# brianz98/A-Fortran-Electronic-Structure-Program

Measured on AMD Instinct MI355X. Metric: CCSD iter wall-time (s) + (T) wall-time (s); fp64 TFLOP/s vs MFMA peak, higher is better.
Workload: dtype f64; 1 GPU; cfg5: nocc=20 nvirt=200, synthetic hashed ERIs scale 0.005; step = 1 CCSD iteration (replicated) + full (T) over i<=j<=k sharded across ranks; nocc=20, nvirt=200, triples=1540, parallelism=(T) ijk-shard x1, CCSD replicas

## Files before the change

### a-fortran-electronic-structure-program_amd/afesp_amd/capi.py

```python
from __future__ import annotations

import ctypes as C
import os

import numpy as np

_HERE = os.path.dirname(os.path.abspath(__file__))
LIB_PATH = os.environ.get("AFESP_LIBRARY") or os.path.join(os.path.dirname(_HERE), "csrc", "libafesp_hip.so")

i64 = C.c_int64
dbl = C.c_double
_dp = np.ctypeslib.ndpointer(dtype=np.float64, flags="C_CONTIGUOUS")
_opt = C.c_void_p

EXPORTS = [
    "afesp_ctx_create", "afesp_ctx_destroy", "afesp_last_error", "afesp_version", "afesp_neri", "afesp_ao2mo_mp2",
    "afesp_ccsd_init", "afesp_ccsd_iterate", "afesp_ccsd_energy", "afesp_ccsd_diis", "afesp_ccsd_solve",
    "afesp_ccsd_get_amplitudes", "afesp_ccsd_set_amplitudes", "afesp_ccsd_get_tensor", "afesp_ccsd_update_intermediates",
    "afesp_ccsd_update_amplitudes", "afesp_ccsd_t_ntriples", "afesp_ccsd_t", "afesp_ccsd_t_shard_bounds", "afesp_gemm", "afesp_permute4",
    "afesp_contract", "afesp_synthetic_init", "afesp_time_pp_ladder", "afesp_bench_contract", "afesp_set_tuning", "afesp_bench_stream", "afesp_profile", "afesp_ccsd_cr_intermediates", "afesp_ccsd_t_cr",
    "afesp_ccsd_so_init", "afesp_ccsd_so_energy", "afesp_ccsd_so_iterate", "afesp_ccsd_so_diis", "afesp_ccsd_so_get_amplitudes",
    "afesp_ccsd_so_set_amplitudes", "afesp_ccsd_so_get_tensor", "afesp_ccsd_so_t_ntriples", "afesp_ccsd_so_t",
    "afesp_read_eri_text", "afesp_write_fcidump", "afesp_set_eri", "afesp_build_fock", "afesp_ccsd_t_plain",
    "afesp_synthetic_ao", "afesp_ccsd_pp_ladder_flop", "afesp_ccsd_iteration_flop",
    "afesp_device_count", "afesp_comm_unique_id", "afesp_comm_init", "afesp_comm_destroy", "afesp_allreduce_sum",
    "afesp_build_fock_uhf", "afesp_ao2mo_ump2", "afesp_ccsd_uso_init", "afesp_mo_window", "afesp_umo_window",
    "afesp_mp2_vv_density", "afesp_ump2_vv_density",
    "afesp_ccsd_t_block_size", "afesp_test_inject", "afesp_ccsd_is_split", "afesp_ccsd_set_split", "afesp_ccsd_set_fused", "afesp_ccsd_iteration_launches", "afesp_debug_stamps", "afesp_launch_counts", "afesp_first_use_count", "afesp_test_ring_path", "afesp_arena_stats",
]
COMM_RCCL, COMM_HOST = 0, 1


class AfespError(RuntimeError):
    pass


_lib = None


def load_library():
    global _lib
    if _lib is not None:
        return _lib
    if not os.path.exists(LIB_PATH):
        raise AfespError(f"{LIB_PATH} is missing: build it with `make -C {os.path.dirname(LIB_PATH)}` "
                         "(there is no CPU fallback for the accelerated path)")
    L = C.CDLL(LIB_PATH)
    L.afesp_ctx_create.argtypes = [C.c_int, C.POINTER(C.c_void_p)]
    L.afesp_ctx_destroy.argtypes = [C.c_void_p]
    L.afesp_ctx_destroy.restype = None
    L.afesp_last_error.argtypes = [C.c_void_p]
    L.afesp_last_error.restype = C.c_char_p
    L.afesp_neri.argtypes = [i64]
    L.afesp_neri.restype = i64
    L.afesp_ao2mo_mp2.argtypes = [C.c_void_p, i64, i64, _dp, _dp, _opt, _opt, C.POINTER(dbl)]
    L.afesp_ccsd_init.argtypes = [C.c_void_p, i64, i64, _opt, _dp, C.c_int]
    L.afesp_ccsd_iterate.argtypes = [C.c_void_p, dbl, dbl, C.POINTER(dbl), C.POINTER(dbl), C.POINTER(C.c_int)]
    L.afesp_ccsd_energy.argtypes = [C.c_void_p, dbl, dbl, C.POINTER(dbl), C.POINTER(dbl), C.POINTER(C.c_int)]
    L.afesp_ccsd_diis.argtypes = [C.c_void_p]
    L.afesp_ccsd_solve.argtypes = [C.c_void_p, C.c_int, dbl, dbl, _dp, _dp, C.POINTER(C.c_int)]
    L.afesp_ccsd_get_amplitudes.argtypes = [C.c_void_p, _dp, _dp]
    L.afesp_ccsd_set_amplitudes.argtypes = [C.c_void_p, _dp, _dp]
    L.afesp_ccsd_get_tensor.argtypes = [C.c_void_p, C.c_char_p, _dp, i64]
    L.afesp_ccsd_update_intermediates.argtypes = [C.c_void_p]
    L.afesp_ccsd_update_amplitudes.argtypes = [C.c_void_p]
    L.afesp_ccsd_t_ntriples.argtypes = [i64]
    L.afesp_ccsd_t_ntriples.restype = i64
    L.afesp_ccsd_t_shard_bounds.argtypes = [C.c_void_p, i64, i64, C.c_int, C.c_int, C.POINTER(i64)]
    L.afesp_ccsd_t.argtypes = [C.c_void_p, i64, i64, _dp]
    L.afesp_ccsd_t_cr.argtypes = [C.c_void_p, i64, i64, _dp]
    L.afesp_ccsd_t_plain.argtypes = [C.c_void_p, i64, i64, _dp]
    L.afesp_ccsd_cr_intermediates.argtypes = [C.c_void_p]
    L.afesp_gemm.argtypes = [C.c_void_p, C.c_char, C.c_char, i64, i64, i64, dbl, _dp, _dp, dbl, _dp]
    L.afesp_permute4.argtypes = [C.c_void_p, C.POINTER(i64), C.c_char_p, _dp, _dp, C.c_int, dbl]
    L.afesp_contract.argtypes = [C.c_void_p, dbl, _dp, C.c_char_p, C.POINTER(i64), _dp, C.c_char_p, C.POINTER(i64), dbl,
                                 _dp, C.c_char_p, C.POINTER(i64), C.c_int, C.c_int, C.c_int]
    L.afesp_synthetic_init.argtypes = [C.c_void_p, i64, i64, dbl, C.c_uint64, C.c_int]
    L.afesp_time_pp_ladder.argtypes = [C.c_void_p, C.c_int, C.POINTER(dbl)]
    L.afesp_synthetic_ao.argtypes = [C.c_void_p, i64, dbl, C.c_uint64]
    L.afesp_ccsd_pp_ladder_flop.argtypes = [C.c_void_p, C.POINTER(dbl)]
    L.afesp_ccsd_iteration_flop.argtypes = [C.c_void_p, C.POINTER(dbl)]
    L.afesp_bench_contract.argtypes = [C.c_void_p, C.c_char_p, C.POINTER(i64), C.c_char_p, C.POINTER(i64), C.c_char_p,
                                       C.POINTER(i64), C.c_int, C.POINTER(dbl)]
    L.afesp_set_tuning.argtypes = [C.c_int, C.c_int, C.c_int, C.c_int]
    L.afesp_bench_stream.argtypes = [C.c_void_p, i64, C.c_int, C.POINTER(dbl)]
    L.afesp_profile.argtypes = [C.c_void_p, C.c_int, _dp]
    L.afesp_ccsd_so_init.argtypes = [C.c_void_p, i64, i64, _opt, _dp, C.c_int, C.c_int]
    L.afesp_ccsd_so_iterate.argtypes = [C.c_void_p, dbl, dbl, C.POINTER(dbl), C.POINTER(dbl), C.POINTER(C.c_int)]
    L.afesp_ccsd_so_energy.argtypes = [C.c_void_p, dbl, dbl, C.POINTER(dbl), C.POINTER(dbl), C.POINTER(C.c_int)]
    L.afesp_ccsd_so_diis.argtypes = [C.c_void_p]
    L.afesp_ccsd_so_get_amplitudes.argtypes = [C.c_void_p, _dp, _dp]
    L.afesp_ccsd_so_set_amplitudes.argtypes = [C.c_void_p, _dp, _dp]
    L.afesp_ccsd_so_get_tensor.argtypes = [C.c_void_p, C.c_char_p, _dp, i64]
    L.afesp_ccsd_so_t_ntriples.argtypes = [i64]
    L.afesp_ccsd_so_t_ntriples.restype = i64
    L.afesp_ccsd_so_t.argtypes = [C.c_void_p, i64, i64, C.POINTER(dbl)]
    L.afesp_read_eri_text.argtypes = [C.c_void_p, C.c_char_p, i64, _opt, C.POINTER(i64)]
    L.afesp_write_fcidump.argtypes = [C.c_void_p, C.c_char_p, i64, C.POINTER(i64)]
    L.afesp_set_eri.argtypes = [C.c_void_p, i64, _dp]
    L.afesp_build_fock.argtypes = [C.c_void_p, i64, _dp, _dp, _dp]
    L.afesp_build_fock_uhf.argtypes = [C.c_void_p, i64, _dp, _dp, _dp, _dp, _dp]
    L.afesp_ao2mo_ump2.argtypes = [C.c_void_p, i64, i64, i64, _dp, _dp, _dp, _dp, _opt, _opt, _opt, _opt, C.POINTER(dbl)]
    L.afesp_ccsd_uso_init.argtypes = [C.c_void_p, i64, i64, i64, _dp, _dp, C.c_int]
    L.afesp_mo_window.argtypes = [C.c_void_p, i64, i64, i64, i64, _dp, _opt, _opt, C.POINTER(dbl)]
    L.afesp_umo_window.argtypes = [C.c_void_p, i64, i64, i64, i64, i64, _dp, _dp, _opt, _opt, _opt, C.POINTER(dbl)]
    L.afesp_mp2_vv_density.argtypes = [C.c_void_p, i64, i64, i64, _dp, _dp, C.POINTER(dbl)]
    L.afesp_ump2_vv_density.argtypes = [C.c_void_p, i64, i64, i64, i64, _dp, _dp, _dp, _dp, C.POINTER(dbl)]
    L.afesp_device_count.argtypes = []
    L.afesp_comm_unique_id.argtypes = [C.c_char_p]
    L.afesp_comm_init.argtypes = [C.c_void_p, C.c_int, C.c_int, C.c_int, C.c_char_p, C.c_char_p]
    L.afesp_comm_destroy.argtypes = [C.c_void_p]
    L.afesp_allreduce_sum.argtypes = [C.c_void_p, _dp, i64]
    L.afesp_ccsd_t_block_size.argtypes = [C.c_void_p, i64, i64, C.c_int, C.POINTER(C.c_int)]
    L.afesp_test_inject.argtypes = [C.c_void_p, C.c_int]
    L.afesp_arena_stats.argtypes = [C.c_void_p, _dp]
    L.afesp_ccsd_is_split.argtypes = [C.c_void_p, C.POINTER(C.c_int)]
    L.afesp_ccsd_set_split.argtypes = [C.c_void_p, C.c_int]
    L.afesp_ccsd_set_fused.argtypes = [C.c_void_p, C.c_int]
    L.afesp_ccsd_iteration_launches.argtypes = [C.c_void_p, C.POINTER(C.c_int)]
    L.afesp_debug_stamps.argtypes = [C.c_void_p, C.c_int]
    L.afesp_launch_counts.argtypes = [C.c_void_p, C.POINTER(C.c_uint64)]
    L.afesp_first_use_count.argtypes = []
    L.afesp_first_use_count.restype = C.c_uint64
    L.afesp_test_ring_path.argtypes = [C.c_int64, C.c_int64]
    _lib = L
    return L


def _f(a):
    return np.ascontiguousarray(np.asarray(a, dtype=np.float64).ravel(order="F"))


TENSOR_SHAPES = {
    "v_oovv": "oovv", "v_ovov": "ovov", "v_vvov": "vvov", "v_oovo": "oovo", "v_oooo": "oooo", "v_vvvv": "vvvv",
    "I_vo": "vo", "I_vv": "vv", "I_oo_p": "oo", "I_oo": "oo", "c_oovv": "oovv", "asym_t2": "oovv", "x_voov": "voov",
    "I_oooo": "oooo", "I_ovov": "ovov", "I_voov": "voov", "I_vovv_p": "vovv", "I_ooov_p": "ooov", "r1": "ov",
    "r2": "oovv", "D1": "ov", "D2": "oovv", "t1": "ov", "t2": "oovv",
}


def device_count():
    return int(load_library().afesp_device_count())


def first_use_count():
    return int(load_library().afesp_first_use_count())


class Engine:

    def __init__(self, device: int = 0):
        self.L = load_library()
        h = C.c_void_p()
        rc = self.L.afesp_ctx_create(device, C.byref(h))
        if rc != 0:
            raise AfespError(f"afesp_ctx_create(device={device}) failed with status {rc} "
                             "(no usable MI355X/HIP device; the accelerated path has no CPU fallback)")
        self.h = h
        self.o = self.v = 0

    def close(self):
        if getattr(self, "h", None):
            self.L.afesp_ctx_destroy(self.h)
            self.h = None

    def __del__(self):
        self.close()

    def __enter__(self):
        return self

    def __exit__(self, *exc):
        self.close()

    def _chk(self, rc):
        if rc != 0:
            raise AfespError(f"status {rc}: {self.L.afesp_last_error(self.h).decode()}")

    def do_mp2_spatial(self, nbasis, nocc, canon_coeff, canon_levels, eri_packed, want_eri_mo=True):
        e2 = dbl(0.0)
        out = np.zeros(self.L.afesp_neri(nbasis)) if want_eri_mo else None
        src = None
        if eri_packed is not None:
            eri_packed = np.ascontiguousarray(eri_packed, dtype=np.float64)
            src = eri_packed.ctypes.data_as(C.c_void_p)
        self._chk(self.L.afesp_ao2mo_mp2(self.h, nbasis, nocc, _f(canon_coeff), _f(canon_levels), src,
                                         out.ctypes.data_as(C.c_void_p) if out is not None else None, C.byref(e2)))
        return e2.value, out

    def ccsd_init(self, nocc, nvirt, canon_levels, eri_mo_packed=None, diis_n_errmat=8):
        self.o, self.v = int(nocc), int(nvirt)
        ptr = None
        if eri_mo_packed is not None:
            eri_mo_packed = np.ascontiguousarray(eri_mo_packed, dtype=np.float64)
            ptr = eri_mo_packed.ctypes.data_as(C.c_void_p)
        self._chk(self.L.afesp_ccsd_init(self.h, nocc, nvirt, ptr, _f(canon_levels), diis_n_errmat))

    def synthetic_init(self, nocc, nvirt, scale=0.02, seed=12345, diis_n_errmat=8):
        self.o, self.v = int(nocc), int(nvirt)
        self._chk(self.L.afesp_synthetic_init(self.h, nocc, nvirt, scale, seed, diis_n_errmat))

    def ccsd_energy(self, e_tol=1e-6, t_tol=1e-7):
        e, r, c = dbl(), dbl(), C.c_int()
        self._chk(self.L.afesp_ccsd_energy(self.h, e_tol, t_tol, C.byref(e), C.byref(r), C.byref(c)))
# ... 4 lines not shown
        self._chk(self.L.afesp_ccsd_iterate(self.h, e_tol, t_tol, C.byref(e), C.byref(r), C.byref(c)))
        return e.value, r.value, bool(c.value)

    def ccsd_diis(self):
        self._chk(self.L.afesp_ccsd_diis(self.h))

    def update_intermediates(self):
        self._chk(self.L.afesp_ccsd_update_intermediates(self.h))

    def update_amplitudes(self):
        self._chk(self.L.afesp_ccsd_update_amplitudes(self.h))

    def do_ccsd_spatial(self, maxiter=50, e_tol=1e-6, t_tol=1e-7):
        en = np.zeros(maxiter + 1)
        rm = np.zeros(maxiter + 1)
        nit = C.c_int()
        self._chk(self.L.afesp_ccsd_solve(self.h, maxiter, e_tol, t_tol, en, rm, C.byref(nit)))
        return nit.value, en, rm

    def amplitudes(self):
        o, v = self.o, self.v
        t1 = np.zeros(o * v)
        t2 = np.zeros(o * o * v * v)
        self._chk(self.L.afesp_ccsd_get_amplitudes(self.h, t1, t2))
        return t1.reshape((o, v), order="F"), t2.reshape((o, o, v, v), order="F")

    def set_amplitudes(self, t1, t2):
        self._chk(self.L.afesp_ccsd_set_amplitudes(self.h, _f(t1), _f(t2)))

    def tensor(self, name):
        dims = tuple(self.o if ch == "o" else self.v for ch in TENSOR_SHAPES[name])
        buf = np.zeros(int(np.prod(dims)))
        self._chk(self.L.afesp_ccsd_get_tensor(self.h, name.encode(), buf, buf.size))
        return buf.reshape(dims, order="F")

    def ntriples(self):
        return self.L.afesp_ccsd_t_ntriples(self.o)

    def shard_bounds(self, world, cr=False):
        b = (i64 * (world + 1))()
        self._chk(self.L.afesp_ccsd_t_shard_bounds(self.h, self.o, self.v, 1 if cr else 0, world, b))
        return [int(x) for x in b]

    def do_ccsd_t_spatial(self, t_begin=0, t_end=None):
        out = np.zeros(4)
        if t_end is None:
            t_end = self.ntriples()
        self._chk(self.L.afesp_ccsd_t(self.h, t_begin, t_end, out))
        return out

    def comm_unique_id(self) -> bytes:
        buf = C.create_string_buffer(128)
        rc = self.L.afesp_comm_unique_id(buf)
        if rc != 0:
            raise AfespError(f"afesp_comm_unique_id failed with status {rc} (is librccl.so.1 loadable?)")
        return buf.raw

    def comm_init(self, rank, world, transport=COMM_RCCL, bootstrap_path=None, unique_id=None):
        self._chk(self.L.afesp_comm_init(self.h, rank, world, transport,
                                         None if bootstrap_path is None else str(bootstrap_path).encode(), unique_id))

    def comm_destroy(self):
        self._chk(self.L.afesp_comm_destroy(self.h))

    def allreduce_sum(self, values):
        buf = np.ascontiguousarray(values, dtype=np.float64).copy()
        self._chk(self.L.afesp_allreduce_sum(self.h, buf, buf.size))
        return buf

    def t_block_size(self, cr=False):
        sb = C.c_int()
        self._chk(self.L.afesp_ccsd_t_block_size(self.h, self.o, self.v, 1 if cr else 0, C.byref(sb)))
        return sb.value

    def arena_stats(self):
        out = np.zeros(4)
        self._chk(self.L.afesp_arena_stats(self.h, out))
        return dict(driver_calls=int(out[0]), reuse_hits=int(out[1]), idle_gb=out[2] / 1e9, live_gb=out[3] / 1e9)

    def launch_counts(self):
        out = (C.c_uint64 * 4)()
        self._chk(self.L.afesp_launch_counts(self.h, out))
        return dict(tall=int(out[0]), gett=int(out[1]), tgemm=int(out[2]), tgemm_mixed=int(out[3]))

    def ccsd_set_split(self, mode):
        self._chk(self.L.afesp_ccsd_set_split(self.h, int(mode)))

    def ccsd_set_fused(self, mode):
        self._chk(self.L.afesp_ccsd_set_fused(self.h, int(mode)))

    def ccsd_iteration_launches(self):
        n = C.c_int()
        self._chk(self.L.afesp_ccsd_iteration_launches(self.h, C.byref(n)))
        return n.value

    def ccsd_is_split(self):
        f = C.c_int()
        self._chk(self.L.afesp_ccsd_is_split(self.h, C.byref(f)))
        return bool(f.value)

    def test_inject(self, what):
        self._chk(self.L.afesp_test_inject(self.h, what))

    def read_eri_text(self, path, nbasis, want_host_copy=True):
        out = np.zeros(self.L.afesp_neri(nbasis)) if want_host_copy else None
        n = i64()
        self._chk(self.L.afesp_read_eri_text(self.h, str(path).encode(), nbasis,
                                             out.ctypes.data_as(C.c_void_p) if out is not None else None, C.byref(n)))
        return out, n.value

    def set_eri(self, nbasis, eri_packed):
        self._chk(self.L.afesp_set_eri(self.h, nbasis, np.ascontiguousarray(eri_packed, dtype=np.float64)))

    def build_fock(self, nbasis, density, core_hamil):
        out = np.zeros(nbasis * nbasis)
        self._chk(self.L.afesp_build_fock(self.h, nbasis, _f(density), _f(core_hamil), out))
        return out.reshape((nbasis, nbasis), order="F")

    def build_fock_uhf(self, nbasis, dens_a, dens_b, core_hamil):
        fa, fb = np.zeros(nbasis * nbasis), np.zeros(nbasis * nbasis)
        self._chk(self.L.afesp_build_fock_uhf(self.h, nbasis, _f(dens_a), _f(dens_b), _f(core_hamil), fa, fb))
        return fa.reshape((nbasis, nbasis), order="F"), fb.reshape((nbasis, nbasis), order="F")

    def do_ump2(self, nbasis, nalpha, nbeta, coeff_a, coeff_b, levels_a, levels_b, eri_packed=None, want_eri_mo=True):
        e2 = dbl(0.0)
        npr = nbasis * (nbasis + 1) // 2
        aa = np.zeros(self.L.afesp_neri(nbasis)) if want_eri_mo else None
        bb = np.zeros(self.L.afesp_neri(nbasis)) if want_eri_mo else None
        ab = np.zeros(npr * npr) if want_eri_mo else None
        src = None
        if eri_packed is not None:
            eri_packed = np.ascontiguousarray(eri_packed, dtype=np.float64)
            src = eri_packed.ctypes.data_as(C.c_void_p)
        ptr = lambda a: a.ctypes.data_as(C.c_void_p) if a is not None else None
        self._chk(self.L.afesp_ao2mo_ump2(self.h, nbasis, nalpha, nbeta, _f(coeff_a), _f(coeff_b),
                                          np.ascontiguousarray(levels_a, dtype=np.float64), np.ascontiguousarray(levels_b, dtype=np.float64),
                                          src, ptr(aa), ptr(ab), ptr(bb), C.byref(e2)))
        return e2.value, aa, (ab.reshape((npr, npr)) if ab is not None else None), bb

    def init_cc_uspinorb(self, nbasis, nalpha, nbeta, levels_a, levels_b, diis_nerr=8):
        self.so_o = int(nalpha + nbeta)
        self.so_v = int(2 * nbasis - self.so_o)
        self._chk(self.L.afesp_ccsd_uso_init(self.h, nbasis, nalpha, nbeta, np.ascontiguousarray(levels_a, dtype=np.float64),
                                             np.ascontiguousarray(levels_b, dtype=np.float64), diis_nerr))

    def mo_window(self, nbasis, nocc, nfc, nfv, canon_levels, eri_mo=None, want_eri=True):
        e2 = dbl(0.0)
        n_act = int(nbasis) - int(nfc) - int(nfv)
        out = np.zeros(self.L.afesp_neri(n_act)) if want_eri and 0 < n_act <= nbasis else None
        src = None
        if eri_mo is not None:
            eri_mo = np.ascontiguousarray(eri_mo, dtype=np.float64)
            src = eri_mo.ctypes.data_as(C.c_void_p)
        self._chk(self.L.afesp_mo_window(self.h, nbasis, nocc, nfc, nfv, np.ascontiguousarray(canon_levels, dtype=np.float64), src,
                                         out.ctypes.data_as(C.c_void_p) if out is not None else None, C.byref(e2)))
        return out, e2.value

    def umo_window(self, nbasis, nalpha, nbeta, nfc, nfv, levels_a, levels_b, want_eri=True):
        e2 = dbl(0.0)
        n_act = int(nbasis) - int(nfc) - int(nfv)
        ok = want_eri and 0 < n_act <= nbasis
        npr = n_act * (n_act + 1) // 2
        aa = np.zeros(self.L.afesp_neri(n_act)) if ok else None
        bb = np.zeros(self.L.afesp_neri(n_act)) if ok else None
        ab = np.zeros(npr * npr) if ok else None
        ptr = lambda a: a.ctypes.data_as(C.c_void_p) if a is not None else None
# ... 193 lines not shown
```

### a-fortran-electronic-structure-program_amd/csrc/afesp_internal.h

```cpp
#pragma once
#include <hip/hip_runtime.h>
#include <stdint.h>

#include <map>
#include <stdexcept>
#include <string>
#include <thread>
#include <vector>

#include "gett.h"
#include "tgemm.h"

namespace afesp {

struct Error : std::runtime_error {
    int code;
    Error(int c, const std::string& m) : std::runtime_error(m), code(c) {}
};

#define AFESP_HIP(expr)                                                                                    \
    do {                                                                                                   \
        hipError_t e_ = (expr);                                                                            \
        if (e_ != hipSuccess)                                                                              \
            throw ::afesp::Error(2, std::string(#expr) + ": " + hipGetErrorString(e_) + " (" + __FILE__ + \
                                        ":" + std::to_string(__LINE__) + ")");                            \
    } while (0)

struct Tensor {
    double* d = nullptr;
    int rank = 0;
    int64_t dim[6] = {0, 0, 0, 0, 0, 0};
    int64_t stride[6] = {0, 0, 0, 0, 0, 0};
    int64_t frozen = 0;
    int64_t size() const
    {
        int64_t s = 1;
        for (int i = 0; i < rank; ++i) s *= dim[i];
        return s;
    }
};

struct Plan {
    int64_t *offAm, *offAk, *offBk, *offBn, *offCm, *offCn;
    int M, N, K;
    bool swapped, a_kc, b_kc, wide;
    bool a_mu = false, b_nu = false;
    int repack = 0;
    int64_t repack_stride[6] = {0, 0, 0, 0, 0, 0};
    int64_t repack_of = 0, repack_epoch = -1;
    const double* repack_src = nullptr;
};

struct Comm;
struct Recorder;

struct Arena {
    std::map<void*, size_t> live;
    std::multimap<size_t, void*> idle;
    size_t idle_bytes = 0, driver_calls = 0, reuse_hits = 0;
    void* get(size_t bytes);
    void* take_largest(size_t min_bytes, size_t max_bytes, size_t* got);
    void put(void* p);
    void trim();
    void destroy();
};

struct Context {
    int device = 0;
    Comm* comm = nullptr;
    int cc_split_mode = -1;
    int test_throw = 0;
    int fused_mode = -1;
    struct PendingTables { int64_t* dst; std::vector<int64_t> img; };
    std::vector<PendingTables> pending_host;
    std::vector<std::vector<int64_t>> pending_merged;
    void plan_uploads_issue();
    void plan_uploads_done() { pending_host.clear(); pending_merged.clear(); }
    Recorder* rec = nullptr;
    hipStream_t stream = nullptr;
    Arena arena;
    std::vector<void*> owned;
    GettWorkspace ws{nullptr, 0};
    TgLaunchState tg;
    unsigned long long n_tall = 0, n_gett = 0;
    bool in_repack = false;
    GettProblem* capture = nullptr;
    struct Lane {
        hipStream_t stream = nullptr;
        GettWorkspace ws{nullptr, 0};
        hipEvent_t done = nullptr;
    };
    std::vector<Lane> lanes;
    size_t lane_ws_bytes = (size_t)8 << 20;
    struct Prepared {
        std::vector<Lane> lanes;
        void* ws_block = nullptr;
        size_t ws_bytes = 0;
    };
    Prepared prepared;
    std::thread startup;
    static void prepare_lanes(Prepared& out, int nlanes);
    hipEvent_t fork_ev = nullptr;
    int cur_lane = 0;
    void fork(int nlanes);
    void use_lane(int i);
    void join();
    int mark();
    void wait(int mark_id);
    std::vector<hipEvent_t> marks;
    int marks_used = 0;
    double* scal = nullptr;
    double* scal_host = nullptr;
    double* res_host = nullptr;
    double* res_dev = nullptr;
    int64_t res_seq = 0;
    int64_t pub_seq = 0;
    std::map<std::string, Plan> plans;
    size_t plan_bytes = 0;
    std::vector<void*> plan_blocks;
    int64_t* plan_slab = nullptr;
    size_t plan_slab_left = 0;
    int64_t* plan_alloc(size_t n);
    void plan_clear();
    int64_t plan_epoch = 0;
    std::map<std::string, std::pair<void*, size_t>> cache;
    std::string last_error;
    bool prof = false;
    double prof_gemm_ms = 0.0, prof_gemm_flop = 0.0, prof_orbit_ms = 0.0, prof_orbit_bytes = 0.0;
    double prof_gemm_flop_padded = 0.0;
    int prof_gemm_kind = 0;
    int64_t prof_gemm_launches = 0, prof_orbit_launches = 0;

    double* alloc(int64_t n);
    double* alloc_raw(int64_t n);
    int64_t* alloc_i64(int64_t n);
    void release(void* p);
    double* scratch(const std::string& name, int64_t ndoubles);
    void drop_scratch();
    void drop_scratch(const std::string& prefix);
    int64_t scratch_epoch = 0;
    int64_t amp_clock = 0;
    const void* t_ops_owner = nullptr;
    int64_t t_ops_amp = -1, t_ops_scratch = -1, t_ops_cr = -1;
    bool t_ops_ts = false;
    Tensor tensor(std::initializer_list<int64_t> dims);
    void sync();
    void quiesce();
    ~Context();
};

Tensor view(double* d, std::initializer_list<int64_t> dims);

void contract(Context& cx, double alpha, const Tensor& A, const char* la, const Tensor& B, const char* lb, double beta,
              const Tensor& C, const char* lc, int nbatch = 1, const int64_t* bA = nullptr, const int64_t* bB = nullptr,
              const int64_t* bC = nullptr, int force_split = 0, int force_tm = 0, int force_tn = 0);

struct ContractCall {
    double alpha;
    const Tensor* A;
    const char* la;
    const Tensor* B;
    const char* lb;
    double beta;
    const Tensor* C;
    const char* lc;
};
void contract_pair(Context& cx, const ContractCall& c1, const ContractCall& c2);
// ... 95 lines not shown
```

### a-fortran-electronic-structure-program_amd/csrc/capi.hip

```cpp
#include <atomic>
#include <chrono>
#include <mutex>
#include <cstdio>
#include <cstring>
#include <thread>
#include <vector>

#include "../../include/afesp.h"
#include "integrals.h"
#include "ccsd_so.h"
#include "comm.h"
#include "fused.h"
#include "tall.h"

using namespace afesp;

struct afesp_ctx {
    Context cx;
    CCState cc;
    SOState so;
    Integrals in;
    struct GraphSlot {
        hipGraphExec_t exec = nullptr;
        int64_t epoch = -1;
        int calls = 0;
        bool disabled = false;
        void reset()
        {
            if (exec) (void)hipGraphExecDestroy(exec);
            exec = nullptr;
            calls = 0;
            disabled = knobs().no_graph;
        }
    } graph_cc;
    FusedSlot fused_int, fused_amp, fused_iter;
    FusedSlot fused_so;
    void cc_programs_reset()
    {
        graph_cc.reset();
        fused_slot_reset(cx, fused_int);
        fused_slot_reset(cx, fused_amp);
        fused_slot_reset(cx, fused_iter);
    }
    void so_programs_reset() { fused_slot_reset(cx, fused_so); }
};

namespace {

struct PreloadClaim {
    std::mutex mu;
    unsigned long long claimed = 0;
    bool claim(int dev)
    {
        std::lock_guard<std::mutex> lk(mu);
        if (dev < 0 || dev >= 64 || (claimed >> dev) & 1ull) return false;
        claimed |= 1ull << dev;
        return true;
    }
};
PreloadClaim g_preload;

template <class F>
int entry(afesp_ctx* c, F&& f)
{
    if (!c) return 1;
    Context& cx = c->cx;
    first_use_tls_device() = cx.device;
    knobs_refresh();
    auto failed = [&](const char* what, int code) {
        cx.last_error = what;
        if (!cx.lanes.empty()) {
            cx.quiesce();
            cx.use_lane(0);
            cx.marks_used = 0;
        }
        return code ? code : 1;
    };
    try {
        AFESP_HIP(hipSetDevice(cx.device));
        f(cx);
        return 0;
    } catch (const Error& e) {
        return failed(e.what(), e.code);
    } catch (const std::exception& e) {
        return failed(e.what(), 1);
    }
}

template <class Body>
double time_on_stream(Context& cx, int reps, Body body)
{
    struct Event { hipEvent_t e = nullptr; ~Event() { if (e) (void)hipEventDestroy(e); } } a, b;
    AFESP_HIP(hipEventCreate(&a.e));
    AFESP_HIP(hipEventCreate(&b.e));
    body();
    AFESP_HIP(hipEventRecord(a.e, cx.stream));
    for (int r = 0; r < reps; ++r) body();
    AFESP_HIP(hipEventRecord(b.e, cx.stream));
    AFESP_HIP(hipEventSynchronize(b.e));
    float ms = 0.f;
    AFESP_HIP(hipEventElapsedTime(&ms, a.e, b.e));
    return (double)ms / (reps > 0 ? reps : 1);
}

__device__ __forceinline__ double hash_uniform(uint64_t x)
{
    x += 0x9E3779B97F4A7C15ull;
    x = (x ^ (x >> 30)) * 0xBF58476D1CE4E5B9ull;
    x = (x ^ (x >> 27)) * 0x94D049BB133111EBull;
    x ^= x >> 31;
    return (double)(x >> 11) * (1.0 / 9007199254740992.0);
}
__global__ void synth_packed_kernel(double* packed, int64_t n, double scale, uint64_t seed)
{
    for (int64_t k = (int64_t)blockIdx.x * blockDim.x + threadIdx.x; k < n; k += (int64_t)gridDim.x * blockDim.x)
        packed[k] = scale * (2.0 * hash_uniform(seed + (uint64_t)k) - 1.0);
}

}

template <typename Body>
static void replay(afesp_ctx* ctx, afesp_ctx::GraphSlot& g, bool eligible, Body body)
{
    Context& cx = ctx->cx;
    if (g.exec && g.epoch != cx.scratch_epoch) {
        (void)hipGraphExecDestroy(g.exec);
        g.exec = nullptr;
        g.calls = 0;
    }
    if (g.exec) {
        AFESP_HIP(hipGraphLaunch(g.exec, cx.stream));
        return;
    }
    if (!eligible || g.disabled) {
        body();
        return;
    }
    const int graph_after = knobs().graph_after;
    if (g.calls == 0 || g.epoch != cx.scratch_epoch || g.calls < graph_after) {
        body();
        g.calls = (g.epoch != cx.scratch_epoch) ? 1 : g.calls + 1;
        g.epoch = cx.scratch_epoch;
        return;
    }
    cx.use_lane(0);
    hipStream_t origin = cx.stream;
    hipGraph_t graph = nullptr;
    if (hipStreamBeginCapture(origin, hipStreamCaptureModeThreadLocal) != hipSuccess) {
        (void)hipGetLastError();
        g.disabled = true;
// ... 54 lines not shown
    replay(ctx, ctx->graph_cc, ccsd_uses_lanes(ctx->cc), [&] {
        ccsd_intermediates(ctx->cx, ctx->cc, true);
        ccsd_amplitudes(ctx->cx, ctx->cc);
        ccsd_energy_launch(ctx->cx, ctx->cc);
    });
    return false;
}

extern "C" {

int afesp_version(void) { return 1; }
int64_t afesp_neri(int64_t nbasis) { return neri_of(nbasis); }

int afesp_ctx_create(int device, afesp_ctx** out)
{
    if (!out) return 1;
    *out = nullptr;
    int ndev = 0;
    if (hipGetDeviceCount(&ndev) != hipSuccess || ndev <= 0) return 10;
    if (device < 0 || device >= ndev) return 11;
    if (hipSetDevice(device) != hipSuccess) return 12;
    afesp_ctx* c = new afesp_ctx();
    c->cx.device = device;
    int rc = entry(c, [&](Context&) {
        AFESP_HIP(hipStreamCreate(&c->cx.stream));
        c->cx.scal = c->cx.alloc(64 + 18 * 512);
        AFESP_HIP(hipHostMalloc((void**)&c->cx.scal_host, sizeof(double) * 64, hipHostMallocDefault));
        AFESP_HIP(hipHostMalloc((void**)&c->cx.res_host, sizeof(double) * (8 + 256 + 72), hipHostMallocCoherent | hipHostMallocMapped));
        memset(c->cx.res_host, 0, sizeof(double) * (8 + 256 + 72));
        AFESP_HIP(hipHostGetDevicePointer((void**)&c->cx.res_dev, c->cx.res_host, 0));
        c->cx.ws.bytes = (size_t)256 << 20;
        c->cx.ws.ptr = c->cx.alloc((int64_t)(c->cx.ws.bytes / sizeof(double)));
        c->cx.sync();
        if (!knobs().no_preload) {
            if (g_preload.claim(device)) c->cx.startup = std::thread([device, c] {
                first_use_tls_device() = device;
                if (hipSetDevice(device) != hipSuccess) return;
                if (knobs().preload_lanes) Context::prepare_lanes(c->cx.prepared, 6);
                {
                    void* d = nullptr;
                    hipStream_t st = nullptr;
                    std::vector<double> h(4096, 1.0);
                    if (hipStreamCreateWithFlags(&st, hipStreamNonBlocking) == hipSuccess && hipMalloc(&d, h.size() * sizeof(double)) == hipSuccess) {
                        (void)hipMemsetAsync(d, 0, h.size() * sizeof(double), st);
                        (void)hipMemcpyAsync(d, h.data(), h.size() * sizeof(double), hipMemcpyHostToDevice, st);
                        (void)hipMemcpyAsync((char*)d + 8192, d, 8192, hipMemcpyDeviceToDevice, st);
                        (void)hipMemcpyAsync(h.data(), d, h.size() * sizeof(double), hipMemcpyDeviceToHost, st);
                        (void)hipStreamSynchronize(st);
                    }
                    if (d) (void)hipFree(d);
                    if (st) (void)hipStreamDestroy(st);
                    (void)hipGetLastError();
                }
                const bool dbg = knobs().preload_debug;
                auto timed = [dbg](const char* what, void (*fn)()) {
                    const auto t0 = std::chrono::steady_clock::now();
                    fn();
                    if (dbg) fprintf(stderr, "afesp preload %-10s %7.2f ms\n", what, std::chrono::duration<double, std::milli>(std::chrono::steady_clock::now() - t0).count());
                };
                timed("kernels", preload_kernels);
                timed("fused", preload_fused);
                timed("contract", preload_contract);
                timed("small path", preload_small_path_kernels);
                timed("triples", preload_triples);
                timed("ccsd_so", preload_ccsd_so);
                timed("uhf", preload_uhf_kernels);
                if (knobs().preload_gett) timed("gett", preload_gett);
            });
        }
    });
    if (rc) {
        if (c->cx.startup.joinable()) c->cx.startup.join();
        delete c;
        return rc;
    }
    *out = c;
    return 0;
}

void afesp_ctx_destroy(afesp_ctx* ctx)
{
    if (!ctx) return;
    first_use_tls_device() = ctx->cx.device;
    (void)hipSetDevice(ctx->cx.device);
    if (ctx->cx.startup.joinable()) ctx->cx.startup.join();
    ctx->cc_programs_reset();
    ctx->so_programs_reset();
    comm_destroy(ctx->cx.comm);
    ctx->cx.comm = nullptr;
    triples_plan_free(ctx->cc);
    so_triples_plan_free(ctx->so);
    ring_free(ctx->cx, ctx->cc);
    delete ctx;
}

const char* afesp_last_error(const afesp_ctx* ctx) { return ctx ? ctx->cx.last_error.c_str() : "null context"; }

int afesp_ao2mo_mp2(afesp_ctx* ctx, int64_t nbasis, int64_t nocc, const double* canon_coeff, const double* canon_levels,
                    const double* eri_packed, double* eri_mo_packed, double* e_mp2)
{
    return entry(ctx, [&](Context& cx) {
        if (nbasis <= 0 || nocc <= 0 || nbasis - nocc <= 0 || nbasis > 1024) throw Error(1, "afesp_ao2mo_mp2: bad extents");
        const double emp2 = ao2mo_mp2(cx, ctx->in, ctx->cc, nbasis, nocc, canon_coeff, canon_levels, eri_packed, eri_mo_packed);
        if (e_mp2) *e_mp2 = emp2;
    });
}

int afesp_mo_window(afesp_ctx* ctx, int64_t nbasis, int64_t nocc, int64_t n_frozen_core, int64_t n_frozen_virt,
                    const double* canon_levels, const double* eri_mo_packed, double* eri_act, double* e_mp2)
{
    return entry(ctx, [&](Context& cx) {
        const int64_t n = nbasis, nfc = n_frozen_core, nfv = n_frozen_virt;
        if (n <= 0 || n > 1024 || nocc <= 0 || nocc >= n || !canon_levels) throw Error(1, "afesp_mo_window: bad extents");
        if (nfc < 0 || nfv < 0) throw Error(1, "afesp_mo_window: negative number of frozen orbitals");
        if (nfc >= nocc) throw Error(1, "afesp_mo_window: no active occupied orbital left");
        if (nfv >= n - nocc) throw Error(1, "afesp_mo_window: no active virtual orbital left");
        if (!eri_mo_packed && (!ctx->in.mo || ctx->in.mo_n != n))
            throw Error(1, "afesp_mo_window: eri_mo_packed is NULL and no MO integrals are resident for this basis size "
                           "(call afesp_ao2mo_mp2 first; a window is taken once)");
        const double emp2 = mo_window(cx, ctx->in, ctx->cc, n, nocc, nfc, nfv, canon_levels, eri_mo_packed, eri_act);
        if (e_mp2) *e_mp2 = emp2;
    });
}

int afesp_mp2_vv_density(afesp_ctx* ctx, int64_t nbasis, int64_t nocc, int64_t n_frozen_core, const double* canon_levels, double* d_vv,
                         double* e_mp2)
{
    return entry(ctx, [&](Context& cx) {
        const int64_t n = nbasis, nfc = n_frozen_core;
        if (n <= 0 || n > 1024 || nocc <= 0 || nocc >= n || !canon_levels || !d_vv) throw Error(1, "afesp_mp2_vv_density: bad extents");
        if (nfc < 0) throw Error(1, "afesp_mp2_vv_density: negative number of frozen orbitals");
        if (nfc >= nocc) throw Error(1, "afesp_mp2_vv_density: no active occupied orbital left");
        if (!ctx->in.mo || ctx->in.mo_n != n)
            throw Error(1, "afesp_mp2_vv_density: no MO integrals are resident for this basis size (call afesp_ao2mo_mp2 first, and "
                           "afesp_mo_window afterwards)");
        const double emp2 = mp2_vv_density(cx, ctx->in, n, nocc, nfc, canon_levels, d_vv);
        if (e_mp2) *e_mp2 = emp2;
    });
}

int afesp_ccsd_init(afesp_ctx* ctx, int64_t nocc, int64_t nvirt, const double* eri_mo_packed, const double* canon_levels,
                    int diis_n_errmat)
{
    return entry(ctx, [&](Context& cx) {
        const int64_t n = nocc + nvirt;
        if (nocc <= 0 || nvirt <= 0 || n > 1024) throw Error(1, "afesp_ccsd_init: bad extents");
        const double* src = ctx->in.mo;
        double* tmp = nullptr;
        if (eri_mo_packed) {
            if (ccsd_can_reinit(ctx->cc, (int)nocc, (int)nvirt, diis_n_errmat) && ctx->cc.eri_own) {
                cx.quiesce();
                if (ctx->cc.eri_src == ctx->cc.eri_own) ctx->cc.eri_src = nullptr;
                cx.release(ctx->cc.eri_own);
                ctx->cc.eri_own = nullptr;
            }
            tmp = cx.alloc(neri_of(n));
            AFESP_HIP(hipMemcpyAsync(tmp, eri_mo_packed, sizeof(double) * neri_of(n), hipMemcpyHostToDevice, cx.stream));
            src = tmp;
        } else if (!src || ctx->in.mo_n != n) {
            throw Error(1, "afesp_ccsd_init: no MO integrals resident for this basis size (call afesp_ao2mo_mp2 first)");
        }
        if (!ccsd_can_reinit(ctx->cc, (int)nocc, (int)nvirt, diis_n_errmat)) {
            ctx->cc_programs_reset();
            cx.drop_scratch("ao2mo_");
        } else {
            ctx->graph_cc.reset();
// ... 676 lines not shown
        cx.sync();
        comm_destroy(cx.comm);
        cx.comm = nullptr;
        ctx->cc_programs_reset();
    });
}

int afesp_allreduce_sum(afesp_ctx* ctx, double* inout, int64_t n)
{
    return entry(ctx, [&](Context& cx) {
        if (n < 0 || (n > 0 && !inout)) throw Error(1, "afesp_allreduce_sum: bad arguments");
        if (!cx.comm) return;
        comm_allreduce_host(cx, cx.comm, inout, n);
    });
}

int afesp_ccsd_is_split(afesp_ctx* ctx, int* split)
{
    return entry(ctx, [&](Context& cx) {
        if (!ctx->cc.ready || !split) throw Error(1, "afesp_ccsd_is_split: no CCSD state");
        ccsd_refresh_sharding(cx, ctx->cc);
        *split = ctx->cc.sharded ? 1 : 0;
    });
}

int afesp_ccsd_set_fused(afesp_ctx* ctx, int mode)
{
    return entry(ctx, [&](Context& cx) {
        if (mode < -1 || mode > 1) throw Error(1, "afesp_ccsd_set_fused: mode is -1 (environment), 0 (call by call) or 1 (launch-fused)");
        cx.fused_mode = mode;
    });
}

int afesp_ccsd_iteration_launches(afesp_ctx* ctx, int* launches)
{
    return entry(ctx, [&](Context& cx) {
        if (!launches) throw Error(1, "afesp_ccsd_iteration_launches: null argument");
        *launches = fused_launches(ctx->fused_iter.prog);
    });
}

int afesp_ccsd_set_split(afesp_ctx* ctx, int mode)
{
    return entry(ctx, [&](Context& cx) {
        if (mode < -1 || mode > 1) throw Error(1, "afesp_ccsd_set_split: mode is -1 (environment), 0 (replicas) or 1 (split)");
        cx.cc_split_mode = mode;
    });
}

int afesp_ccsd_t_block_size(afesp_ctx* ctx, int64_t nocc, int64_t nvirt, int cr, int* block_size)
{
    return entry(ctx, [&](Context& cx) {
        if (nocc < 1 || nvirt < 1 || !block_size) throw Error(1, "afesp_ccsd_t_block_size: bad arguments");
        *block_size = triples_block_size((int)nocc, (int)nvirt, cr != 0);
    });
}

int afesp_debug_stamps(unsigned long long* out, int n)
{
    knobs_refresh();
    if (n < 0) return triples_read_orbit_stamps(out, -n) == hipSuccess ? 0 : 1;
    if (knobs().stamps_grouped) return gett_read_stamps_grouped(out, n) == hipSuccess ? 0 : 1;
    return gett_read_stamps(out, n) == hipSuccess ? 0 : 1;
}

int afesp_test_ring_path(int64_t nocc, int64_t nvirt)
{
    knobs_refresh();
    CCState s;
    s.o = (int)nocc;
    s.v = (int)nvirt;
    return ring_tg_applies(s) ? 1 : 0;
}

uint64_t afesp_first_use_count(void) { return first_use_count().load(std::memory_order_relaxed); }

int afesp_launch_counts(afesp_ctx* ctx, uint64_t out[4])
{
    return entry(ctx, [&](Context& cx) {
        out[0] = cx.n_tall; out[1] = cx.n_gett; out[2] = cx.tg.launches; out[3] = cx.tg.launches_mixed;
    });
}

int afesp_arena_stats(afesp_ctx* ctx, double out[4])
{
    return entry(ctx, [&](Context& cx) {
        const Arena& a = cx.arena;
        size_t live = 0;
        for (auto& kv : a.live) live += kv.second;
        out[0] = (double)a.driver_calls; out[1] = (double)a.reuse_hits; out[2] = (double)a.idle_bytes; out[3] = (double)live;
    });
}

int afesp_test_inject(afesp_ctx* ctx, int what)
{
    return entry(ctx, [&](Context& cx) { cx.test_throw = what; });
}

}
```

### a-fortran-electronic-structure-program_amd/csrc/ccsd.hip

```cpp
#include <algorithm>
#include <cmath>
#include <cstdlib>
#include <cstring>

#include "ccsd.h"
#include "comm.h"
#include "fused.h"

namespace afesp {

static inline int64_t tri64(int64_t i, int64_t j) { return i >= j ? i * (i + 1) / 2 + j : j * (j + 1) / 2 + i; }

bool ccsd_can_reinit(const CCState& s, int o, int v, int diis_nerr)
{
    if (!knobs().cc_reinit) return false;
    return s.ready && s.o == o && s.v == v && s.nerr == diis_nerr && s.pp_sym == pp_sym_pays(o, v);
}

void ccsd_init(Context& cx, CCState& s, int o, int v, const double* eri_mo_dev, const double* e_host, int diis_nerr)
{
    if (o <= 0 || v <= 0) throw Error(1, "ccsd_init: need at least one occupied and one virtual orbital");
    const bool again = ccsd_can_reinit(s, o, v, diis_nerr);
    if (again) {
        cx.quiesce();
// ... 214 lines not shown
    s.amps_touched = false;
    s.r1x_valid = false;
    int64_t v0, v1;
    slice_bounds(s, &v0, &v1);
    auto sl = [&](const Tensor& t, int axis) { return slice_axis(t, axis, v0, v1); };
    if (!(lanes_pay(s) || cx.rec) && ring_tg_applies(s) && ring_tg_pack(cx, s)) {}
    else k_asym_c(cx, s.asym.d, s.c.d, s.t1.d, s.t2.d, s.o, s.v);
    const bool par = lanes_pay(s) && !cx.rec;
    const bool fused = cx.rec != nullptr;
    const bool ring = !par && !fused && ring_tg_applies(s);
    if (!ring) ring_invalidate(s);
    auto lane = [&](int i) { if (par) cx.use_lane(i); };
    if (par) cx.fork(6);
    lane(0);
    C(1.0, s.w_oovv, "miea", s.t1, "me", 0.0, s.I_vo, "ai");
    lane(1);
    const bool ivv_diag = !par && !fused && s.o >= 2;
    if (!ivv_diag) {
        ccsd_need_w_vvov(cx, s);
        C(1.0, s.w_vvov, "ebma", s.t1, "me", 0.0, s.I_vv, "ba");
    }
    if (!s.sharded) C(-1.0, s.w_oovv, "mneb", s.c, "mnea", ivv_diag ? 0.0 : 1.0, s.I_vv, "ba");
    else if (v1 > v0) C(-1.0, s.w_oovv, "mneb", sl(s.c, 3), "mnea", ivv_diag ? 0.0 : 1.0, slice_axis(s.I_vv, 1, v0, v1), "ba");
    lane(0);
    C(1.0, s.w_oovo, "miej", s.t1, "me", 0.0, s.I_oo_p, "ji");
    C(1.0, s.asym, "mjef", s.v_oovv, "mief", 1.0, s.I_oo_p, "ji");
    if (fused) {
        C(1.0, s.w_oovo, "miej", s.t1, "me", 0.0, s.I_oo, "ji");
        C(1.0, s.asym, "mjef", s.v_oovv, "mief", 1.0, s.I_oo, "ji");
    } else {
        k_copy(cx, s.I_oo.d, s.I_oo_p.d, s.I_oo.size());
    }
    C(1.0, s.t1, "je", s.I_vo, "ei", 1.0, s.I_oo, "ji");
    lane(1);
    k_copy(cx, s.I_oooo.d, s.v_oooo.d, s.I_oooo.size());
    if (s.pp_sym && !par && !fused) ccsd_oooo_pair_form(cx, s);
    else C(1.0, s.c, "klef", s.v_oovv, "ijef", 1.0, s.I_oooo, "klij");
    C(1.0, s.t1, "ke", s.v_oovo, "ilej", 1.0, s.I_oooo, "klij");
    C(1.0, s.t1, "le", s.v_oovo, "jkei", 1.0, s.I_oooo, "klij");
    lane(2);
    const int64_t a_len = s.I_ovov.stride[3], a_off = v0 * a_len, a_cnt = (v1 - v0) * a_len;
    if (ivv_diag && s.sharded) {
        if (v1 > v0) C(1.0, s.t1, "je", sl(s.v_vvov, 3), "ebia", 0.0, sl(s.I_ovov, 3), "jbia");
    } else if (ivv_diag) {
        contract_pair(cx, {1.0, &s.t1, "je", &s.v_vvov, "ebia", 0.0, &s.I_ovov, "jbia"}, {1.0, &s.v_vvov, "beia", &s.t1, "je", 0.0, &s.x_voov, "bjia"});
    } else if (v1 > v0) {
        k_copy(cx, s.I_ovov.d + a_off, s.v_ovov.d + a_off, a_cnt);
        if (!ring) C(-0.5, s.v_oovv, "mibe", sl(s.c, 2), "mjae", 1.0, sl(s.I_ovov, 3), "jbia");
        C(-1.0, s.v_oovo, "mibj", sl(s.t1, 1), "ma", 1.0, sl(s.I_ovov, 3), "jbia");
        C(1.0, s.t1, "je", sl(s.v_vvov, 3), "ebia", 1.0, sl(s.I_ovov, 3), "jbia");
    }
    lane(3);
    if (s.sharded) { if (v1 > v0) C(1.0, sl(s.v_vvov, 3), "beia", s.t1, "je", 0.0, sl(s.x_voov, 3), "bjia"); }
    else if (!ivv_diag) C(1.0, s.v_vvov, "beia", s.t1, "je", 0.0, s.x_voov, "bjia");
    if (ivv_diag && v1 > v0) {
        k_ivv_diag(cx, s.I_vv.d, s.I_ovov.d, s.x_voov.d, s.o, s.v, (int)v0, (int)v1);
        k_axpby(cx, s.I_ovov.d + a_off, 1.0, s.v_ovov.d + a_off, 1.0, a_cnt);
        if (!ring) C(-0.5, s.v_oovv, "mibe", sl(s.c, 2), "mjae", 1.0, sl(s.I_ovov, 3), "jbia");
        C(-1.0, s.v_oovo, "mibj", sl(s.t1, 1), "ma", 1.0, sl(s.I_ovov, 3), "jbia");
    }
    const int x_voov_ready = par ? cx.mark() : 0;
    if (v1 > v0) {
        permute_add(cx, 1.0, sl(s.v_oovv, 2), "jiab", 0.0, sl(s.I_voov, 3), "bjia");
        if (fused) C(1.0, s.v_vvov, "beia", s.t1, "je", 1.0, s.I_voov, "bjia");
        else k_axpby(cx, s.I_voov.d + a_off, 1.0, s.x_voov.d + a_off, 1.0, a_cnt);
        if (!ring) {
            C(0.5, s.w_oovv, "imbe", sl(s.t2, 3), "mjea", 1.0, sl(s.I_voov, 3), "bjia");
            C(-0.5, s.v_oovv, "imbe", sl(s.c, 2), "mjae", 1.0, sl(s.I_voov, 3), "bjia");
        }
        C(-1.0, s.v_oovo, "imbj", sl(s.t1, 1), "ma", 1.0, sl(s.I_voov, 3), "bjia");
    }
    if (ring) ring_tg_intermediates(cx, s);
    lane(4);
    if (save_for_diis) diis_save(cx, s);
    if (fused) permute_add(cx, 1.0, s.v_oovo, "kjai", 0.0, s.z_ooov, "jkia");
    C(1.0, s.t1, "ie", s.v_oovv, "mjeb", fused ? 1.0 : 0.0, s.z_ooov, "ijmb");
    C(1.0, s.t1, "je", s.v_ovov, "mbie", 1.0, s.z_ooov, "ijmb");
    lane(5);
    permute_add(cx, 1.0, s.v_oovo, "kjai", 0.0, s.I_ooov_p, "jkia");
    if (s.sharded) {
        Tensor osh = view(cx.scratch("ooov_sh", s.I_ooov_p.size()), {(int64_t)s.o, (int64_t)s.o, (int64_t)s.o, (int64_t)s.v});
        if (v1 > v0) {
            if (s.pp_sym) {
                AFESP_HIP(hipMemsetAsync(osh.d + osh.stride[3] * v0, 0, sizeof(double) * osh.stride[3] * (v1 - v0), cx.stream));
                ccsd_ooov_pair_form(cx, s, osh.d, v0, v1);
            } else {
                C(1.0, s.t2, "jkef", sl(s.v_vvov, 3), "efia", 0.0, sl(osh, 3), "jkia");
            }
            if (par) cx.wait(x_voov_ready);
            C(1.0, s.t1, "je", sl(s.x_voov, 3), "ekia", 1.0, sl(osh, 3), "jkia");
        }
    } else if (s.pp_sym) {
        ccsd_ooov_pair_form(cx, s);
    } else {
        C(1.0, s.t2, "jkef", s.v_vvov, "efia", 1.0, s.I_ooov_p, "jkia");
    }
    if (par) cx.wait(x_voov_ready);
    if (!s.sharded) C(1.0, s.t1, "je", s.x_voov, "ekia", 1.0, s.I_ooov_p, "jkia");
    if (par) cx.join();
    if (fused) {
        C(1.0, s.t2, "jkef", s.v_vvov, "efia", 1.0, s.z_ooov, "jkia");
        C(1.0, s.t1, "je", s.x_voov, "ekia", 1.0, s.z_ooov, "jkia");
    } else {
        k_axpby(cx, s.z_ooov.d, 1.0, s.I_ooov_p.d, 1.0, s.z_ooov.size());
    }
}

static int tile_cols(int64_t n)
{
    if (n <= 32) return 32;
    if (n <= 64) return 64;
    const int64_t wide = (n + 127) / 128 * 128, n7 = (int64_t)((double)((n + 111) / 112 * 112) / 0.93), n6 = (int64_t)((double)((n + 95) / 96 * 96) / 0.93);
    return (int)std::min(wide, std::min(n7, n6));
}
bool pp_sym_pays(int64_t O, int64_t V)
{
    if (knobs().pp_sym >= 0) return knobs().pp_sym == 1;
    const double plain = (double)tile_cols(O * O) * (double)(V * V) * (double)(V * (V + 1) / 2);
    const double split = (double)tile_cols(O * (O + 1) / 2) * (double)(V * (V + 1) / 2) * (double)(V * (V + 1) / 2) +
                         (double)tile_cols(O * (O - 1) / 2) * (double)(V * (V - 1) / 2) * (double)(V * (V - 1) / 2);
    return plain > 1.5 * split;
}

static void pp_b_range(const CCState& s, int64_t* b0, int64_t* b1)
{
    const int64_t V = s.v;
    if (!s.sharded) { *b0 = 0; *b1 = V; return; }
    auto cut = [&](int r) { return (int64_t)std::llround(std::sqrt((double)r / (double)s.sh_world) * (double)V); };
    *b0 = s.sh_rank == 0 ? 0 : std::min(V, cut(s.sh_rank));
    *b1 = s.sh_rank + 1 == s.sh_world ? V : std::min(V, cut(s.sh_rank + 1));
}

static void ccsd_oooo_pair_form(Context& cx, CCState& s)
{
    const int64_t ks = s.pp_ks, ka = s.pp_ka, ns = s.pp_ns, na = s.pp_na, nm = s.pp_nm, kx = s.pp_lds;
    const int64_t* t = s.pp_tab;
    const int64_t* u = t + s.pp_kn;
    k_c_sympack(cx, s.pp_cs, s.pp_ca, s.c.d, s.o, s.v, ns, na);
    s.cs_packed = true;
    GettProblem gp;
    gp.alpha = 1.0; gp.beta = 0.0;
    gp.nbatch = 1; gp.batchA = gp.batchB = gp.batchC = nullptr;
    gp.a_kcontig = false; gp.b_kcontig = false;
    gp.wide = true;
    gp.offAm = gp.offBn = gp.offCm = t;
    gp.A = s.pp_cs; gp.B = s.oo_vs; gp.C = s.oo_xs;
    gp.offAk = gp.offBk = u + 2 * nm; gp.offCn = u + 2 * nm + 2 * kx;
    gp.M = gp.N = (int)ns; gp.K = (int)ks;
    AFESP_HIP(gett_launch(gp, cx.ws, cx.stream));
    if (s.pp_pa) {
        gp.A = s.pp_ca; gp.B = s.oo_va; gp.C = s.oo_xa;
        gp.offAk = gp.offBk = u + 2 * nm + kx; gp.offCn = u + 3 * nm + 2 * kx;
        gp.M = gp.N = (int)na; gp.K = (int)ka;
        AFESP_HIP(gett_launch(gp, cx.ws, cx.stream));
    }
    k_oooo_pair_expand_add(cx, s.I_oooo.d, s.oo_xs, s.pp_pa ? s.oo_xa : nullptr, s.o, ns, na);
}

void ccsd_pp_ladder(Context& cx, CCState& s)
{
    const int64_t O = s.o, V = s.v, np = V * (V + 1) / 2, K2 = V * V, N2 = O * O;
    int64_t b0, b1;
    pp_b_range(s, &b0, &b1);
    const int64_t p0 = b0 * (b0 + 1) / 2, p1 = b1 * (b1 + 1) / 2, q0 = b0 * (b0 - 1) / 2, q1 = b1 * (b1 - 1) / 2;
    GettProblem gp;
    gp.alpha = 1.0; gp.beta = 0.0;
// ... 21 lines not shown
        if (s.pp_pa) k_rows_append(cx, s.pp_va, s.pp_lda, ka, s.pp_ca, na, npa);
        k_oooo_sympack(cx, s.pp_cs + ns * ks, s.pp_pa ? s.pp_ca + na * ka : nullptr, s.I_oooo.d, s.o, ns, na);
    }
    gp.wide = true;
    gp.offAk = t; gp.offBn = gp.offCn = t;
    gp.A = s.pp_vs; gp.B = s.pp_cs; gp.C = s.pp_ps;
    gp.offAm = u + p0; gp.offBk = u + 2 * nm; gp.offCm = u + 2 * nm + 2 * kx + p0;
    gp.M = (int)(p1 - p0); gp.N = (int)ns; gp.K = (int)(fold ? ks + ns : ks);
    const int* pt = knobs().pp_tiles;
    if (cx.rec) cx.rec->product(gp, s.pp_lds * np, ns * ks, ns * np);
    else if (p1 > p0) AFESP_HIP(gett_launch(gp, cx.ws, cx.stream, pt[2], pt[0], pt[1]));
    if (s.pp_pa) {
        gp.A = s.pp_va; gp.B = s.pp_ca; gp.C = s.pp_pa;
        gp.offAm = u + nm + q0; gp.offBk = u + 2 * nm + kx; gp.offCm = u + 3 * nm + 2 * kx + q0;
        gp.M = (int)(q1 - q0); gp.N = (int)na; gp.K = (int)(fold ? ka + na : ka);
        if (cx.rec) cx.rec->product(gp, s.pp_lda * npa, na * ka, na * npa);
        else if (q1 > q0) AFESP_HIP(gett_launch(gp, cx.ws, cx.stream, pt[5], pt[3], pt[4]));
    }
    (void)npa;
    k_pp_expand(cx, s.pp, s.pp_ps, s.pp_pa, s.o, s.v, ns, na, p0, p1);
}

void ccsd_ooov_pair_form(Context& cx, CCState& s, double* out, int64_t a0, int64_t a1)
{
    if (!out) { out = s.I_ooov_p.d; a0 = 0; a1 = s.v; }
    if (a1 <= a0) return;
    const int64_t O = s.o, V = s.v, np = V * (V + 1) / 2, npa = V * (V - 1) / 2, ks = s.pp_ks, ka = s.pp_ka, ns = s.pp_ns, na = s.pp_na,
                  nm = s.pp_nm, M = O * (a1 - a0), m0 = O * a0;
    const int64_t* t = s.pp_tab;
    const int64_t* u = t + s.pp_kn;
    k_c_sympack(cx, s.pp_ts, s.pp_ta, s.t2.d, s.o, s.v, ns, na);
    const int64_t kx = s.pp_lds;
    GettProblem gp;
    gp.alpha = 1.0; gp.beta = 0.0;
    gp.nbatch = 1; gp.batchA = gp.batchB = gp.batchC = nullptr;
    gp.a_kcontig = true; gp.b_kcontig = false;
    gp.wide = true;
    gp.offAk = t; gp.offBn = gp.offCn = t;
    auto slices = [&](int64_t n, int64_t k) {
        if (M >= 2048) return 0;
        const int64_t tiles = ((M + 255) / 256) * ((n + 127) / 128), ksteps = (k + 15) / 16;
        int64_t sp = (256 + tiles - 1) / tiles;
        while (sp > 1 && ksteps / sp < 32) --sp;
        return (int)std::max<int64_t>(1, std::min<int64_t>(sp, 32));
    };
    gp.A = s.ov_ws; gp.B = s.pp_ts; gp.C = s.pp_ps;
    gp.offAm = u + m0; gp.offBk = u + 2 * nm; gp.offCm = u + 2 * nm + 2 * kx + m0;
    gp.M = (int)M; gp.N = (int)ns; gp.K = (int)ks;
    if (cx.rec) cx.rec->product(gp, s.pp_lds * O * V, ns * ks, ns * O * V);
    else AFESP_HIP(gett_launch(gp, cx.ws, cx.stream, slices(ns, ks)));
    if (s.ov_wa) {
        gp.A = s.ov_wa; gp.B = s.pp_ta; gp.C = s.pp_pa;
        gp.offAm = u + nm + m0; gp.offBk = u + 2 * nm + kx; gp.offCm = u + 3 * nm + 2 * kx + m0;
        gp.M = (int)M; gp.N = (int)na; gp.K = (int)ka;
        if (cx.rec) cx.rec->product(gp, s.pp_lda * O * V, na * ka, na * O * V);
        else AFESP_HIP(gett_launch(gp, cx.ws, cx.stream, slices(na, ka)));
    }
    (void)np; (void)npa;
    k_pair_expand_add(cx, out + O * O * m0, s.pp_ps + ns * m0, s.ov_wa ? s.pp_pa + na * m0 : nullptr, s.o, M, ns, na);
    if (out == s.I_ooov_p.d && M == O * V && !cx.rec) {
        k_ooov_r1_trace(cx, s.r1x, s.pp_ps, s.ov_wa ? s.pp_pa : nullptr, s.o, s.v, ns, na);
        s.r1x_valid = true;
    }
}

void ccsd_amplitudes(Context& cx, CCState& s, bool defer_update)
{
    auto C = [&](double al, const Tensor& A, const char* la, const Tensor& B, const char* lb, double be, const Tensor& Cc,
                 const char* lc) { contract(cx, al, A, la, B, lb, be, Cc, lc); };
    ccsd_refresh_sharding(cx, s);
    const bool par = lanes_pay(s) && !cx.rec, sh = s.sharded;
    const bool ring = !par && !cx.rec && !sh && ring_live(s);
    s.partials_live = par;
    ring_res_clear(s);
    int64_t v0, v1;
    slice_bounds(s, &v0, &v1);
    auto sl = [&](const Tensor& t, int axis) { return slice_axis(t, axis, v0, v1); };
    auto lane = [&](int i) { if (par) cx.use_lane(i); };
    Tensor r2b = s.r2, r2c = s.r2, r1b = s.r1;
    Tensor r2s = s.r2;
    if (sh) {
        r2s.d = s.r2_sh;
        const int64_t np = (int64_t)s.v * (s.v + 1) / 2;
        AFESP_HIP(hipMemsetAsync(s.pp, 0, sizeof(double) * ((int64_t)s.o * s.o * np + s.r2.size() + s.r1.size()), cx.stream));
    }
    if (par) {
        r2b.d = cx.scratch("r2_lane2", s.r2.size());
        r2c.d = cx.scratch("r2_lane3", s.r2.size());
        r1b.d = cx.scratch("r1_lane5", s.r1.size());
        cx.fork(6);
    }
    lane(0);
    if (!sh) C(1.0, s.t1, "ie", s.I_vv, "ea", 0.0, s.r1, "ia");
    C(-1.0, s.I_oo_p, "im", s.t1, "ma", sh ? 0.0 : 1.0, s.r1, "ia");
    C(1.0, s.asym, "miea", s.I_vo, "em", 1.0, s.r1, "ia");
    C(2.0, s.v_oovv, "miea", s.t1, "me", 1.0, s.r1, "ia");
    lane(5);
    if (par && cx.test_throw == 1) {
        cx.test_throw = 0;
        throw Error(99, "injected failure (afesp_test_inject)");
    }
    C(-1.0, s.v_ovov, "maie", s.t1, "me", par ? 0.0 : 1.0, r1b, "ia");
    C(-1.0, s.v_oovo, "mien", s.asym, "mnea", 1.0, r1b, "ia");
    if (!sh && s.r1x_valid && !par && !cx.rec) k_axpby(cx, r1b.d, 1.0, s.r1x, 1.0, r1b.size());
    else if (!sh) C(1.0, s.asym, "mief", s.v_vvov, "efma", 1.0, r1b, "ia");
    lane(1);
    const bool open_with_vvov = !par && !cx.rec && !sh;
    if (ring) ring_tg_residual(cx, s);
    if (open_with_vvov && !s.amps_touched) permute_add(cx, 1.0, s.x_voov, "bija", ring ? 1.0 : 0.0, s.r2, "ijab");
    else if (open_with_vvov) C(1.0, s.t1, "ie", s.v_vvov, "baje", ring ? 1.0 : 0.0, s.r2, "ijab");
    if (!sh) {
        C(1.0, s.t2, "ijae", s.I_vv, "eb", open_with_vvov ? 1.0 : 0.0, s.r2, "ijab");
        C(-1.0, s.t2, "miba", s.I_oo, "jm", 1.0, s.r2, "ijab");
    }
    lane(4);
    ccsd_pp_ladder(cx, s);
    lane(1);
    if (!sh && !(s.pp_sym && !cx.rec)) C(0.5, s.I_oooo, "ijmn", s.c, "mnab", 1.0, s.r2, "ijab");
    lane(2);
    if (ring) {
    } else if (!sh) {
        C(-1.0, s.t2, "mjae", s.I_ovov, "iemb", par ? 0.0 : 1.0, r2b, "ijab");
        C(-1.0, s.I_ovov, "iema", s.t2, "mjeb", 1.0, r2b, "ijab");
    } else if (v1 > v0) {
        C(-1.0, s.t2, "mjae", sl(s.I_ovov, 3), "iemb", 1.0, sl(r2s, 3), "ijab");
        C(-1.0, sl(s.I_ovov, 3), "iema", s.t2, "mjeb", 1.0, sl(r2s, 2), "ijab");
        C(1.0, s.asym, "miea", sl(s.I_voov, 3), "ejmb", 1.0, sl(r2s, 3), "ijab");
        Tensor osh = view(cx.scratch("ooov_sh", s.I_ooov_p.size()), {(int64_t)s.o, (int64_t)s.o, (int64_t)s.o, (int64_t)s.v});
        C(-1.0, s.t1, "ma", sl(osh, 3), "ijmb", 1.0, sl(r2s, 3), "ijab");
        C(1.0, s.t1, "ie", slice_axis(s.v_vvov, 0, v0, v1), "baje", 1.0, sl(r2s, 3), "ijab");
        C(1.0, s.t2, "ijae", slice_axis(s.I_vv, 1, v0, v1), "eb", 1.0, sl(r2s, 3), "ijab");
        C(-1.0, slice_axis(s.t2, 2, v0, v1), "miba", s.I_oo, "jm", 1.0, sl(r2s, 3), "ijab");
        C(0.5, s.I_oooo, "ijmn", sl(s.c, 3), "mnab", 1.0, sl(r2s, 3), "ijab");
        C(-1.0, s.t1, "ma", sl(s.z_ooov, 3), "ijmb", 1.0, sl(r2s, 3), "ijab");
        Tensor r1s = s.r1;
        r1s.d = s.r1_sh;
        C(1.0, s.t1, "ie", slice_axis(s.I_vv, 1, v0, v1), "ea", 1.0, slice_axis(r1s, 1, v0, v1), "ia");
        C(1.0, s.asym, "mief", sl(s.v_vvov, 3), "efma", 1.0, slice_axis(r1s, 1, v0, v1), "ia");
    }
    lane(3);
    if (!sh && !ring) C(1.0, s.asym, "miea", s.I_voov, "ejmb", par ? 0.0 : 1.0, r2c, "ijab");
    if (!open_with_vvov && !sh) C(1.0, s.t1, "ie", s.v_vvov, "baje", 1.0, r2c, "ijab");
    if (!sh) C(-1.0, s.t1, "ma", s.z_ooov, "ijmb", 1.0, r2c, "ijab");
    if (par) cx.join();
    if (sh) {
        const int64_t np = (int64_t)s.v * (s.v + 1) / 2;
        comm_allreduce_dev(cx, cx.comm, s.pp, (int64_t)s.o * s.o * np + s.r2.size() + s.r1.size());
        k_copy(cx, s.r2.d, s.r2_sh, s.r2.size());
        k_axpby(cx, s.r1.d, 1.0, s.r1_sh, 1.0, s.r1.size());
    }
    if (defer_update) return;
    k_t2_update(cx, s.t2.d, s.r2.d, par ? r2b.d : nullptr, par ? r2c.d : nullptr, s.v_oovv.d, s.D2.d, s.pp, s.o, s.v, s.t1.d, s.r1.d,
                par ? r1b.d : nullptr, s.D1.d, ring ? ring_Y(s) : nullptr);
}

void ccsd_build_I_vovv_p(Context& cx, CCState& s, const Tensor& out)
{
    permute_add(cx, 1.0, s.v_vvov, "baic", 0.0, out, "ciab");
    contract(cx, -1.0, s.v_oovv, "micb", s.t1, "ma", 1.0, out, "ciab");
    contract(cx, -1.0, s.v_ovov, "maic", s.t1, "mb", 1.0, out, "ciab");
}

void ccsd_tail_launch(Context& cx, CCState& s)
{
    auto launch = [](Context& c, CCState* st) {
        CCTail a;
// ... 105 lines not shown
    k_copy(cx, xovov_pp.d, s.v_ovov.d, xovov_pp.size());
    C(-1.0, s.v_oovo, "mibj", s.t1, "ma", 1.0, xovov_pp, "jbia");
    C(0.5, s.t1, "je", xv, "beai", 1.0, xovov_pp, "jbia");
    permute_add(cx, 1.0, s.v_oovv, "ijba", 0.0, xvoov_p, "bjia");
    C(-0.5, s.v_oovo, "imbj", s.t1, "ma", 1.0, xvoov_p, "bjia");
    C(1.0, xvp, "ebai", s.t1, "je", 1.0, xvoov_p, "bjia");
    permute_add(cx, 1.0, s.v_oovv, "ijba", 0.0, xvoov_pp, "bjia");
    C(-1.0, s.v_oovo, "imbj", s.t1, "ma", 1.0, xvoov_pp, "bjia");
    C(0.5, xv, "ebai", s.t1, "je", 1.0, xvoov_pp, "bjia");
    permute_add(cx, 1.0, s.v_oovo, "jiak", 0.0, xovoo, "kaij");
    C(1.0, s.t1, "ke", s.v_oovv, "ijea", 1.0, xovoo, "kaij");
    permute_add(cx, 1.0, s.v_vvov, "baic", 0.0, s.I_vovv_pp, "ciab");
    ccsd_need_vvvv(cx, s);
    C(1.0, s.v_vvvv, "ecba", s.t1, "ie", 1.0, s.I_vovv_pp, "ciab");
    C(-1.0, xovov_p, "icma", s.t1, "mb", 1.0, s.I_vovv_pp, "ciab");
    C(-1.0, s.t1, "ma", xvoov_p, "cimb", 1.0, s.I_vovv_pp, "ciab");
    C(-1.0, s.I_vo, "cm", s.t2, "miab", 1.0, s.I_vovv_pp, "ciab");
    C(1.0, s.t2, "mnba", xovoo, "icmn", 1.0, s.I_vovv_pp, "ciab");
    C(1.0, xv, "ceam", s.asym, "imbe", 1.0, s.I_vovv_pp, "ciab");
    C(-1.0, xv, "ecam", s.t2, "mieb", 1.0, s.I_vovv_pp, "ciab");
    C(-1.0, s.t2, "miae", xv, "ecbm", 1.0, s.I_vovv_pp, "ciab");
    permute_add(cx, 1.0, s.v_oovo, "kjai", 0.0, s.I_ooov_pp, "jkia");
    C(-1.0, s.v_oooo, "mikj", s.t1, "ma", 1.0, s.I_ooov_pp, "jkia");
    C(1.0, xovov_pp, "jeia", s.t1, "ke", 1.0, s.I_ooov_pp, "jkia");
    C(1.0, s.t1, "je", xvoov_pp, "ekia", 1.0, s.I_ooov_pp, "jkia");
    C(1.0, s.t2, "kjef", xv, "efai", 1.0, s.I_ooov_pp, "jkia");
    const int64_t eb = std::min(O, V);
    auto clip = [](Tensor t, int axis, int64_t n) { t.dim[axis] = n; return t; };
    Tensor xo_e = clip(xovoo, 1, eb), as_e = clip(s.asym, 2, eb), t2_e2 = clip(s.t2, 2, eb), t2_e3 = clip(s.t2, 3, eb);
    C(1.0, xo_e, "jeim", as_e, "mkea", 1.0, s.I_ooov_pp, "jkia");
    C(-1.0, xo_e, "jemi", t2_e2, "mkea", 1.0, s.I_ooov_pp, "jkia");
    C(-1.0, t2_e3, "mjae", xo_e, "kemi", 1.0, s.I_ooov_pp, "jkia");
}

void ccsd_diis_update(Context& cx, CCState& s) { diis_update(cx, s); }

void diis_update(Context& cx, DiisRing& s)
{
    if (s.nerr < 2) return;
    if (s.tail_pending) {
        s.tail_pending = false;
        s.it = s.tail_slot + 1;
        s.nact = s.tail_n;
        const int n = s.nact, N = n + 1;
        double A[17][18];
        for (int i = 0; i < N; ++i)
            for (int j = 0; j <= N; ++j)
                A[i][j] = (i < n && j < n) ? s.tail_b[i + 16 * j] : (j == N) ? (i == n ? -1.0 : 0.0) : (i == n && j == n) ? 0.0 : -1.0;
        for (int k = 0; k < N; ++k) {
            int p = k;
            for (int i = k + 1; i < N; ++i)
                if (std::fabs(A[i][k]) > std::fabs(A[p][k])) p = i;
            if (A[p][k] == 0.0) throw Error(4, "ccsd::update_diis_cc: Linear solve failed!");
            if (p != k)
                for (int j = 0; j <= N; ++j) std::swap(A[k][j], A[p][j]);
            for (int i = k + 1; i < N; ++i) {
                const double f = A[i][k] / A[k][k];
                for (int j = k; j <= N; ++j) A[i][j] -= f * A[k][j];
            }
        }
        double c[17];
        for (int k = N - 1; k >= 0; --k) {
            double r = A[k][N];
            for (int j = k + 1; j < N; ++j) r -= A[k][j] * c[j];
            c[k] = r / A[k][k];
        }
        k_lincomb_vals(cx, s.amp, s.hist_t, s.nvec, c, n, s.nvec);
        return;
    }
    s.it += 1;
    if (s.it > s.nerr) s.it -= s.nerr;
    if (s.nact < s.nerr) s.nact += 1;
    const int slot = s.it - 1, n = s.nact;
    double* ht = s.hist_t + (int64_t)slot * s.nvec;
    double* he = s.hist_e + (int64_t)slot * s.nvec;
    k_diis_push(cx, ht, he, s.amp, s.amp_s, s.hist_e, s.nvec, n, slot, s.nvec);
    k_diis_solve(cx, s.coef, s.bmat, cx.scal + DIIS_FLAG_SLOT, n, s.nerr, slot);
    k_lincomb(cx, s.amp, s.hist_t, s.nvec, s.coef, n, s.nvec);
}

void diis_check_flag(Context& cx, const double* host_scal)
{
    if (host_scal[DIIS_FLAG_SLOT] != 0.0) {
        AFESP_HIP(hipMemsetAsync(cx.scal + DIIS_FLAG_SLOT, 0, sizeof(double), cx.stream));
        throw Error(4, "ccsd::update_diis_cc: Linear solve failed!");
    }
}

}
```

### a-fortran-electronic-structure-program_amd/csrc/contract.hip

```cpp
#include <algorithm>
#include <cstring>

#include "afesp_internal.h"
#include "fused.h"
#include "tall.h"

namespace afesp {

static size_t arena_round(size_t bytes)
{
    if (bytes < 256) bytes = 256;
    const size_t g = bytes >= ((size_t)1 << 20) ? ((size_t)2 << 20) : 256;
    return (bytes + g - 1) / g * g;
}
void* Arena::get(size_t bytes)
{
    bytes = arena_round(bytes);
    auto it = idle.lower_bound(bytes);
    if (it != idle.end() && it->first <= bytes + std::max(bytes / 4, (size_t)1 << 20)) {
        void* p = it->second;
        live[p] = it->first;
        idle_bytes -= it->first;
        idle.erase(it);
        ++reuse_hits;
// ... 110 lines not shown
}
void Context::release(void* p)
{
    if (!p) return;
    auto it = std::find(owned.begin(), owned.end(), p);
    if (it != owned.end()) {
        owned.erase(it);
        quiesce();
        arena.put(p);
    }
}
int64_t* Context::plan_alloc(size_t n)
{
    n = (n + 1) & ~(size_t)1;
    constexpr size_t SLAB = (size_t)1 << 19;
    if (n > SLAB / 4) {
        void* p = arena.get(n * sizeof(int64_t));
        plan_blocks.push_back(p);
        return (int64_t*)p;
    }
    if (plan_slab_left < n) {
        plan_slab = (int64_t*)arena.get(SLAB * sizeof(int64_t));
        plan_blocks.push_back(plan_slab);
        plan_slab_left = SLAB;
    }
    int64_t* p = plan_slab;
    plan_slab += n;
    plan_slab_left -= n;
    return p;
}
void Context::plan_uploads_issue()
{
    std::vector<PendingTables*> v;
    for (auto& t : pending_host)
        if (t.dst && !t.img.empty()) v.push_back(&t);
    std::sort(v.begin(), v.end(), [](const PendingTables* a, const PendingTables* b) { return a->dst < b->dst; });
    for (size_t i = 0; i < v.size();) {
        size_t j = i + 1;
        int64_t* end = v[i]->dst + v[i]->img.size();
        while (j < v.size() && v[j]->dst == end) { end += v[j]->img.size(); ++j; }
        if (j == i + 1) {
            AFESP_HIP(hipMemcpyAsync(v[i]->dst, v[i]->img.data(), v[i]->img.size() * sizeof(int64_t), hipMemcpyHostToDevice, stream));
        } else {
            std::vector<int64_t> merged;
            merged.reserve((size_t)(end - v[i]->dst));
            for (size_t k = i; k < j; ++k) merged.insert(merged.end(), v[k]->img.begin(), v[k]->img.end());
            pending_merged.push_back(std::move(merged));
            AFESP_HIP(hipMemcpyAsync(v[i]->dst, pending_merged.back().data(), pending_merged.back().size() * sizeof(int64_t), hipMemcpyHostToDevice, stream));
        }
        for (size_t k = i; k < j; ++k) v[k]->dst = nullptr;
        i = j;
    }
}
void Context::plan_clear()
{
    if (stream) (void)hipStreamSynchronize(stream);
    for (void* p : plan_blocks) arena.put(p);
    plan_blocks.clear();
    plan_slab = nullptr;
    plan_slab_left = 0;
    plans.clear();
    plan_bytes = 0;
    ++plan_epoch;
}

Tensor Context::tensor(std::initializer_list<int64_t> dims)
{
    int64_t n = 1;
    for (auto d : dims) n *= d;
    return view(alloc(n), dims);
}
void Context::sync() { AFESP_HIP(hipStreamSynchronize(stream)); }

void Context::fork(int nlanes)
{
    if (cur_lane != 0) throw Error(1, "Context::fork: already forked");
    if (startup.joinable()) startup.join();
    if (lanes.empty()) {
        lanes.resize(1);
        lanes[0].stream = stream;
        lanes[0].ws = ws;
        AFESP_HIP(hipEventCreateWithFlags(&fork_ev, hipEventDisableTiming));
    }
    if (lanes.size() == 1 && !prepared.lanes.empty()) {
        if (prepared.ws_block) {
            arena.live[prepared.ws_block] = prepared.ws_bytes;
            owned.push_back(prepared.ws_block);
        }
        for (Lane& l : prepared.lanes) lanes.push_back(l);
        prepared.lanes.clear();
        prepared.ws_block = nullptr;
    }
    for (size_t i = 1; i < lanes.size(); ++i)
        if (lanes[i].ws.bytes < lane_ws_bytes) {
            void* p = arena.get(lane_ws_bytes);
            owned.push_back(p);
            lanes[i].ws.ptr = (double*)p;
            lanes[i].ws.bytes = lane_ws_bytes;
        }
    while ((int)lanes.size() < nlanes) {
        Lane l;
        AFESP_HIP(hipStreamCreateWithFlags(&l.stream, hipStreamNonBlocking));
        AFESP_HIP(hipEventCreateWithFlags(&l.done, hipEventDisableTiming));
        l.ws.bytes = lane_ws_bytes;
        void* p = arena.get(l.ws.bytes);
        owned.push_back(p);
        l.ws.ptr = (double*)p;
        lanes.push_back(l);
    }
    AFESP_HIP(hipEventRecord(fork_ev, lanes[0].stream));
    for (size_t i = 1; i < lanes.size(); ++i) AFESP_HIP(hipStreamWaitEvent(lanes[i].stream, fork_ev, 0));
}

void Context::prepare_lanes(Prepared& out, int nlanes)
{
    const size_t each = (size_t)8 << 20;
    void* block = nullptr;
    if (nlanes < 2 || hipMalloc(&block, each * (size_t)(nlanes - 1)) != hipSuccess) {
        (void)hipGetLastError();
        return;
    }
    out.ws_block = block;
    out.ws_bytes = each * (size_t)(nlanes - 1);
    for (int i = 1; i < nlanes; ++i) {
        Lane l;
        if (hipStreamCreateWithFlags(&l.stream, hipStreamNonBlocking) != hipSuccess ||
            hipEventCreateWithFlags(&l.done, hipEventDisableTiming) != hipSuccess) {
            (void)hipGetLastError();
            break;
        }
        l.ws.ptr = (double*)((char*)block + each * (size_t)(i - 1));
        l.ws.bytes = each;
        out.lanes.push_back(l);
    }
}

void Context::use_lane(int i)
{
    if (lanes.empty()) return;
    cur_lane = i % (int)lanes.size();
    stream = lanes[(size_t)cur_lane].stream;
    ws = lanes[(size_t)cur_lane].ws;
}

int Context::mark()
{
    if (marks_used == (int)marks.size()) {
        hipEvent_t e;
        AFESP_HIP(hipEventCreateWithFlags(&e, hipEventDisableTiming));
        marks.push_back(e);
    }
    AFESP_HIP(hipEventRecord(marks[(size_t)marks_used], stream));
    return marks_used++;
}

void Context::wait(int mark_id) { AFESP_HIP(hipStreamWaitEvent(stream, marks[(size_t)mark_id], 0)); }

void Context::join()
{
    marks_used = 0;
    if (lanes.empty()) return;
    for (size_t i = 1; i < lanes.size(); ++i) {
        AFESP_HIP(hipEventRecord(lanes[i].done, lanes[i].stream));
        AFESP_HIP(hipStreamWaitEvent(lanes[0].stream, lanes[i].done, 0));
    }
    use_lane(0);
}
Context::~Context()
{
    if (startup.joinable()) startup.join();
    use_lane(0);
    for (size_t i = 1; i < lanes.size(); ++i) {
        (void)hipStreamSynchronize(lanes[i].stream);
        (void)hipStreamDestroy(lanes[i].stream);
        (void)hipEventDestroy(lanes[i].done);
    }
    for (Lane& l : prepared.lanes) {
        (void)hipStreamDestroy(l.stream);
        (void)hipEventDestroy(l.done);
    }
    if (prepared.ws_block) (void)hipFree(prepared.ws_block);
    if (fork_ev) (void)hipEventDestroy(fork_ev);
    for (hipEvent_t e : marks) (void)hipEventDestroy(e);
    if (stream) (void)hipStreamSynchronize(stream);
    arena.destroy();
    if (scal_host) (void)hipHostFree(scal_host);
    if (res_host) (void)hipHostFree(res_host);
    tgemm_state_free(tg);
    if (stream) (void)hipStreamDestroy(stream);
}

Tensor view(double* d, std::initializer_list<int64_t> dims)
{
    Tensor t;
    t.d = d;
    t.rank = (int)dims.size();
    int64_t s = 1;
    int i = 0;
    for (auto x : dims) {
        t.dim[i] = x;
        t.stride[i] = s;
        s *= x;
        ++i;
    }
    return t;
}

__global__ void publish_scalars_kernel(double* __restrict__ dst, const double* __restrict__ src, int n, double seq)
{
    if ((int)threadIdx.x < n) dst[threadIdx.x] = src[threadIdx.x];
    __threadfence_system();
    __syncthreads();
    if (threadIdx.x == 0) __hip_atomic_store(&dst[64], seq, __ATOMIC_RELEASE, __HIP_MEMORY_SCOPE_SYSTEM);
}

double* host_scalars(Context& cx, int n)
{
    hipStreamCaptureStatus st = hipStreamCaptureStatusNone;
    if (n > 64 || !cx.res_dev || hipStreamIsCapturing(cx.stream, &st) != hipSuccess || st != hipStreamCaptureStatusNone) {
        (void)hipGetLastError();
        AFESP_HIP(hipMemcpyAsync(cx.scal_host, cx.scal, sizeof(double) * n, hipMemcpyDeviceToHost, cx.stream));
        cx.sync();
        return cx.scal_host;
    }
    constexpr int PUB = 8 + 256;
    const double want = (double)++cx.pub_seq;
    AFESP_KLAUNCH(publish_scalars_kernel, dim3(1), dim3(64), 0, cx.stream, cx.res_dev + PUB, cx.scal, n, want);
    AFESP_HIP(hipGetLastError());
    return host_scalars_wait(cx, n, want);
}

double* host_scalars_slot(Context& cx, double* seq)
{
    hipStreamCaptureStatus st = hipStreamCaptureStatusNone;
    if (!cx.res_dev || hipStreamIsCapturing(cx.stream, &st) != hipSuccess || st != hipStreamCaptureStatusNone) {
        (void)hipGetLastError();
        return nullptr;
    }
    *seq = (double)++cx.pub_seq;
    return cx.res_dev + 8 + 256;
}

double* host_scalars_wait(Context& cx, int n, double want)
{
    constexpr int PUB = 8 + 256;
    bool seen = false;
    for (int spin = 0; spin < 400000; ++spin) {
        if (__atomic_load_n((const int64_t*)&cx.res_host[PUB + 64], __ATOMIC_ACQUIRE) == *(const int64_t*)&want) { seen = true; break; }
        if ((spin & 1023) == 1023 && hipStreamQuery(cx.stream) != hipErrorNotReady) break;
    }
    if (!seen) {
        AFESP_HIP(hipStreamSynchronize(cx.stream));
        if (cx.res_host[PUB + 64] != want) throw Error(2, "host_scalars: the published values did not arrive");
    }
    for (int q = 0; q < n; ++q) cx.scal_host[q] = cx.res_host[PUB + q];
    return cx.scal_host;
}

namespace {

struct Lab {
    char c;
    int64_t dim;
    int64_t sa, sb, sc;
};

int64_t stride_of(const Tensor& t, const char* l, char c)
{
    for (int i = 0; i < t.rank; ++i)
        if (l[i] == c) return t.stride[i];
    return -1;
}

char min_stride_label(const Tensor& t, const char* l)
{
    char best = 0;
    int64_t bs = INT64_MAX;
    for (int i = 0; i < t.rank; ++i)
        if (t.dim[i] > 1 && t.stride[i] < bs) {
            bs = t.stride[i];
            best = l[i];
        }
    if (!best && t.rank > 0) best = l[0];
    return best;
}

std::vector<int64_t> table(const std::vector<Lab>& g, int which)
{
    int64_t n = 1;
    for (auto& l : g) n *= l.dim;
    std::vector<int64_t> t((size_t)n);
    std::vector<int64_t> idx(g.size(), 0);
    for (int64_t x = 0; x < n; ++x) {
        int64_t off = 0;
        for (size_t q = 0; q < g.size(); ++q) off += idx[q] * (which == 0 ? g[q].sa : which == 1 ? g[q].sb : g[q].sc);
        t[(size_t)x] = off;
        for (size_t q = 0; q < g.size(); ++q) {
            if (++idx[q] < g[q].dim) break;
            idx[q] = 0;
        }
    }
    return t;
}
// ... 520 lines not shown
```

### a-fortran-electronic-structure-program_amd/csrc/first_use.h

```cpp
#pragma once
#include <hip/hip_runtime.h>
#include <stdint.h>

#include "knobs.h"

#include <atomic>
#include <mutex>

namespace afesp {

inline std::mutex& first_use_mutex()
{
    static std::mutex m;
    return m;
}
inline int& first_use_tls_device()
{
    static thread_local int dev = -1;
    return dev;
}
inline uint64_t first_use_bit()
{
    int d = first_use_tls_device();
    if (d < 0 && hipGetDevice(&d) != hipSuccess) d = 0;
    return (uint64_t)1 << (d & 63);
}
inline void first_use_touch(const void* fn)
{
    std::lock_guard<std::mutex> lk(first_use_mutex());
    hipFuncAttributes at;
    (void)hipFuncGetAttributes(&at, fn);
    (void)hipGetLastError();
}
inline void first_use_resolve(const void* fn, std::atomic<uint64_t>& seen, uint64_t bit)
{
    first_use_touch(fn);
    seen.fetch_or(bit, std::memory_order_release);
}
inline std::atomic<uint64_t>& first_use_count()
{
    static std::atomic<uint64_t> n{0};
    return n;
}

}

#define AFESP_KLAUNCH(kernel, grid, block, shmem, stream, ...)                                                          \
    do {                                                                                                                \
        static std::atomic<uint64_t> afesp_seen_{0};                                                                    \
        const uint64_t afesp_bit_ = ::afesp::first_use_bit();                                                           \
        if (!(afesp_seen_.load(std::memory_order_acquire) & afesp_bit_)) {                                              \
            ::afesp::first_use_resolve(reinterpret_cast<const void*>(kernel), afesp_seen_, afesp_bit_);                 \
            ::afesp::first_use_count().fetch_add(1, std::memory_order_relaxed);                                         \
        }                                                                                                               \
        kernel<<<(grid), (block), (shmem), (stream)>>>(__VA_ARGS__);                                                    \
    } while (0)
```

### a-fortran-electronic-structure-program_amd/csrc/fused.hip

```cpp
#include <algorithm>
#include <cstdio>
#include <cstdlib>
#include <cstring>
#include <map>

#include "fused.h"

namespace afesp {

typedef double v4d __attribute__((ext_vector_type(4)));

struct FItem {
    const double* A;
    const double* B;
    double* P;
    const int64_t *offAm, *offBn, *offCm, *offCn;
    const uint32_t* kofs;
    int M, N, K, m0, n0, k0, k1, tile;
    double alpha;
    int64_t pad[3];
};
static_assert(sizeof(FItem) == 128, "FItem is read as two s_load_dwordx16");
struct EwOp {
    double* out;
// ... 125 lines not shown
        }
}

__global__ __launch_bounds__(256, 2) void fused_gemm_kernel(const FItem* __restrict__ items, int nitems)
{
    const int w = (int)blockIdx.x * 4 + __builtin_amdgcn_readfirstlane((int)threadIdx.x >> 6);
    if (w >= nitems) return;
    const FItem it = items[w];
    const int lane = threadIdx.x & 63;
    switch (it.tile) {
        case 0: fused_tile<1, 1, 4>(it, lane); break;
        case 1: fused_tile<2, 2, 3>(it, lane); break;
        case 2: fused_tile<4, 1, 3>(it, lane); break;
        case 3: fused_tile<1, 4, 3>(it, lane); break;
        case 4: fused_tile<1, 1, 2>(it, lane); break;
        case 5: fused_tile<2, 2, 2>(it, lane); break;
        case 6: fused_tile<4, 1, 2>(it, lane); break;
        default: fused_tile<1, 4, 2>(it, lane); break;
    }
}

__global__ __launch_bounds__(256) void fused_ew_kernel(const EwOp* __restrict__ ops, const EwBlk* __restrict__ blks)
{
    const EwBlk b = blks[blockIdx.x];
    const EwOp& op = ops[b.op];
    const int rank = op.rank, nsum = op.nsum, gshift = op.gshift, G = 1 << gshift;
    const int64_t n = op.n, sstride = op.sstride;
    const double alpha = op.alpha, beta = op.beta;
    double* __restrict__ out = op.out;
    const double* __restrict__ in = op.in;
#pragma unroll
    for (int t = 0; t < EW_PER_BLOCK / 256; ++t) {
        const int tid = t * 256 + threadIdx.x;
        const int64_t x = b.x0 + (tid >> gshift);
        const int g = tid & (G - 1);
        const bool live = x < n;
        int64_t oo = x, io = x;
        if (rank > 1 && live) {
            int64_t r = x;
            oo = io = 0;
            for (int q = 0; q < rank; ++q) {
                const int64_t i = r % op.dim[q];
                r /= op.dim[q];
                oo += i * op.so[q];
                io += i * op.si[q];
            }
        }
        double s = 0.0;
        if (live) {
            int q = g;
            for (; q + 3 * G < nsum; q += 4 * G) {
                const double l0 = in[io + (int64_t)q * sstride], l1 = in[io + (int64_t)(q + G) * sstride],
                             l2 = in[io + (int64_t)(q + 2 * G) * sstride], l3 = in[io + (int64_t)(q + 3 * G) * sstride];
                s += l0; s += l1; s += l2; s += l3;
            }
            for (; q < nsum; q += G) s += in[io + (int64_t)q * sstride];
        }
        for (int off = G >> 1; off > 0; off >>= 1) s += __shfl_down(s, off, 64);
        if (live && g == 0) {
            double val = alpha * s;
            if (beta != 0.0) val += beta * out[oo];
            out[oo] = val;
        }
    }
}

void preload_fused()
{
    first_use_touch(reinterpret_cast<const void*>(fused_gemm_kernel));
    first_use_touch(reinterpret_cast<const void*>(fused_ew_kernel));
    first_use_touch(reinterpret_cast<const void*>(build_kofs_kernel));
    (void)hipGetLastError();
}

void Recorder::product(const GettProblem& g, int64_t a_span, int64_t b_span, int64_t c_span)
{
    if (g.nbatch != 1 || g.batchA || g.batchB || g.batchC) return fail("batched product");
    if (g.M <= 0 || g.N <= 0 || g.K <= 0) return fail("empty product");
    const double big = knobs().fused_big_flop;
    if (2.0 * g.M * (double)g.N * g.K >= big || a_span >= ((int64_t)1 << 28) || b_span >= ((int64_t)1 << 28) || c_span >= ((int64_t)1 << 28)) {
        std::vector<FusedRange> rd = {frange(g.A, a_span), frange(g.B, b_span)};
        if (g.beta != 0.0) rd.push_back(frange(g.C, c_span));
        const GettProblem gp = g;
        opaque(rd, {frange(g.C, c_span)}, [gp](Context& c) { AFESP_HIP(gett_launch(gp, c.ws, c.stream)); }, 2);
        ops.back().heavy = true;
        return;
    }
    if ((int64_t)g.M * g.N != c_span) return fail("product into a strided view");
    Op o;
    o.kind = PRODUCT;
    o.g = g;
    o.c_span = c_span;
    o.reads = {frange(g.A, a_span), frange(g.B, b_span)};
    if (g.beta != 0.0) o.reads.push_back(frange(g.C, c_span));
    o.writes = {frange(g.C, c_span)};
    ops.push_back(std::move(o));
}

void Recorder::elementwise(double* out, const double* in, int rank, const int64_t* dim, const int64_t* so, const int64_t* si, double alpha,
                           double beta)
{
    if (rank > 6) return fail("elementwise rank > 6");
    Op o;
    o.kind = ELEMENTWISE;
    o.out = out;
    o.in = in;
    o.alpha = alpha;
    o.beta = beta;
    int64_t ospan = 1, ispan = 1;
    for (int q = 0; q < rank; ++q) {
        if (dim[q] == 1) continue;
        ospan += (dim[q] - 1) * so[q];
        ispan += (dim[q] - 1) * si[q];
        if (o.rank > 0 && so[q] == o.so[o.rank - 1] * o.dim[o.rank - 1] && si[q] == o.si[o.rank - 1] * o.dim[o.rank - 1]) {
            o.dim[o.rank - 1] *= dim[q];
        } else {
            o.dim[o.rank] = dim[q]; o.so[o.rank] = so[q]; o.si[o.rank] = si[q];
            ++o.rank;
        }
    }
    if (o.rank == 0) { o.rank = 1; o.dim[0] = 1; o.so[0] = o.si[0] = 1; }
    if (o.rank == 1 && (o.so[0] != 1 || o.si[0] != 1)) { o.dim[1] = 1; o.so[1] = o.si[1] = 0; o.rank = 2; }
    o.reads = {frange(in, ispan)};
    if (beta != 0.0) o.reads.push_back(frange(out, ospan));
    o.writes = {frange(out, ospan)};
    ops.push_back(std::move(o));
}

void Recorder::opaque(std::vector<FusedRange> reads, std::vector<FusedRange> writes, std::function<void(Context&)> fn, int nlaunch)
{
    Op o;
    o.kind = OPAQUE;
    o.reads = std::move(reads);
    o.writes = std::move(writes);
    o.fn = std::move(fn);
    o.nlaunch = nlaunch;
    ops.push_back(std::move(o));
}

struct FusedProgram {
    struct Stage {
        int kind = 0;
        const FItem* items = nullptr;
        int nitems = 0;
        const EwOp* ewops = nullptr;
        const EwBlk* blks = nullptr;
        int nblk = 0;
        std::vector<std::function<void(Context&)>> opaque;
        std::vector<std::function<void(Context&)>> heavy;
        std::vector<std::pair<int, int>> per_op;
    };
    std::vector<Stage> stages;
    void* desc = nullptr;
    double* slabs = nullptr;
    uint32_t* ktab = nullptr;
    int64_t epoch = 0;
    int64_t plan_epoch = 0;
    int launches = 0;
};

namespace {

bool overlap(const std::vector<FusedRange>& a, const std::vector<FusedRange>& b)
{
    for (auto& x : a)
        for (auto& y : b)
            if (x.lo < y.hi && y.lo < x.hi) return true;
// ... 360 lines not shown
```

### a-fortran-electronic-structure-program_amd/csrc/gett.h

```cpp
#pragma once
#include <hip/hip_runtime.h>
#include "first_use.h"
#include <stdint.h>

namespace afesp {

struct GettProblem {
    const double* A;
    const double* B;
    double* C;
    const int64_t* offAm;
    const int64_t* offAk;
    const int64_t* offBk;
    const int64_t* offBn;
    const int64_t* offCm;
    const int64_t* offCn;
    int M, N, K;
    double alpha, beta;
    int nbatch;
    const int64_t* batchA;
    const int64_t* batchB;
    const int64_t* batchC;
    bool a_kcontig, b_kcontig;
    bool wide = false;
    bool a_munit = false, b_nunit = false;
};

struct GettGroup {
    int64_t a_off;
    const int64_t* offAk;
    const int64_t* offBk;
    const int64_t* offBn;
    const int64_t* offCn;
    int N, ntiles, tile_start, pad;
};
void gett_grouped_tile(int M, bool wide, int* tm, int* tn, int* BM, int* BN);
hipError_t gett_launch_grouped(const GettProblem& p, const GettGroup* dev_groups, int ngroups, int total_tiles, int max_ntiles,
                               hipStream_t stream);

struct GettWorkspace {
    double* ptr;
    size_t bytes;
};

hipError_t gett_launch(const GettProblem& p, const GettWorkspace& ws, hipStream_t stream, int force_split = 0,
                       int force_tm = 0, int force_tn = 0);

hipError_t gett_read_stamps(unsigned long long* out, int n);
hipError_t gett_read_stamps_grouped(unsigned long long* out, int n);
void preload_gett_grouped();

extern int g_group_m, g_force_tm, g_force_tn, g_force_split, g_allow_wide, g_dbg;

}
```

### a-fortran-electronic-structure-program_amd/csrc/gett.hip

```cpp
#include "gett.h"

#include <cstdio>
#include <cstdlib>

namespace afesp {

typedef double v4d __attribute__((ext_vector_type(4)));

static __device__ unsigned long long g_gett_stamp[256 * 8 * 4];

constexpr int BK = 16;

#ifndef AFESP_GETT_VARIANT
#define AFESP_GETT_VARIANT 0
#endif
#define AFESP_GETT_VARIANT_ (AFESP_GETT_VARIANT)

typedef double v2d __attribute__((ext_vector_type(2)));

template <int BMN, bool KC, int NT, int W>
struct TileImg {
    static constexpr int LD = KC ? (BK + 2) : (BMN + 16);
    static constexpr int SIZE = KC ? BMN * LD : BK * LD;
    static constexpr int PER = BMN * BK / (NT * W);
// ... 10 lines not shown
    static constexpr int NKO = KC ? 1 : T::PER;
    int64_t rowoff[NROW];
    int64_t ko[NKO];
    const double* base;
    const int64_t* offK;
    int K;

    __device__ __forceinline__ void init(const double* X, const int64_t* offMN, const int64_t* offK_, int mn0, int MN,
                                         int K_, int t)
    {
        base = X;
        offK = offK_;
        K = K_;
#pragma unroll
        for (int r = 0; r < NROW; ++r) {
            int mn = mn0 + T::mn_of(t, r);
            rowoff[r] = offMN[mn < MN ? mn : MN - (KC ? 1 : W)];
        }
    }
    __device__ __forceinline__ void rows(const int64_t* offMN, int mn0, int MN, int t)
    {
#pragma unroll
        for (int r = 0; r < NROW; ++r) {
            int mn = mn0 + T::mn_of(t, r);
            rowoff[r] = offMN[mn < MN ? mn : MN - (KC ? 1 : W)];
        }
    }
    __device__ __forceinline__ void fetch_ko(int k0, int t)
    {
#pragma unroll
        for (int r = 0; r < NKO; ++r) {
            int k = k0 + T::k_of(t, r);
            ko[r] = offK[k < K ? k : K - W];
        }
    }
    __device__ __forceinline__ void fetch(double (&reg)[T::PER][W]) const
    {
#pragma unroll
        for (int r = 0; r < T::PER; ++r) {
            const double* src = base + rowoff[KC ? r : 0] + ko[KC ? 0 : r];
            if (W == 2) {
                const v2d x = *reinterpret_cast<const v2d*>(src);
                reg[r][0] = x[0];
                reg[r][W - 1] = x[1];
            } else {
                reg[r][0] = *src;
            }
        }
    }
    __device__ __forceinline__ void stash(double* s, const double (&reg)[T::PER][W], int t, int k0, int kend, bool tail) const
    {
#pragma unroll
        for (int r = 0; r < T::PER; ++r) {
            const int mn = T::mn_of(t, r), k = T::k_of(t, r);
            double x0 = reg[r][0], x1 = reg[r][W - 1];
            if (tail) {
                x0 = (k0 + k < kend) ? x0 : 0.0;
                x1 = (k0 + k + (KC ? W - 1 : 0) < kend) ? x1 : 0.0;
            }
            if (W == 2) *reinterpret_cast<v2d*>(&s[T::at(mn, k)]) = (v2d){x0, x1};
            else s[T::at(mn, k)] = x0;
        }
    }
};

__device__ __forceinline__ int uniform_i32(int x) { return __builtin_amdgcn_readfirstlane(x); }
__device__ __forceinline__ int64_t uniform_i64(int64_t x)
{
    const int lo = __builtin_amdgcn_readfirstlane((int)x), hi = __builtin_amdgcn_readfirstlane((int)(x >> 32));
    return ((int64_t)hi << 32) | (unsigned)lo;
}
template <typename T>
__device__ __forceinline__ const T* uniform_ptr(const T* p)
{
    typedef const T __attribute__((address_space(1)))* gptr;
    return (const T*)reinterpret_cast<gptr>(uniform_i64(reinterpret_cast<int64_t>(p)));
}

struct GettKernelArgs {
    GettProblem p;
    int ksplit;
    int kchunk;
    double* ws;
    int mtiles, ntiles;
    int gm;
    int dbg;
    const GettGroup* groups;
    int total_tiles;
    int sk_units;
    int sk_nk;
};

__device__ __forceinline__ int xcd_remap(int b, int nwg)
{
    int q = nwg >> 3, r = nwg & 7, xcd = b & 7;
    return (xcd < r ? xcd * (q + 1) : r * (q + 1) + (xcd - r) * q) + (b >> 3);
}

template <int WM, int WN, int TM, int TN, bool AKC, bool BKC, int W, bool GRP = false, bool RAG = !GRP, int TS = TN, bool SK = false>
__global__ __launch_bounds__(64 * WM * WN, (WM * WN == 4 && TM * TN < 16 && !(AFESP_GETT_VARIANT_ & 2048)) ? 2 : 1) void gett_kernel(GettKernelArgs a)
{
    constexpr int NT = 64 * WM * WN;
    constexpr int BM = 16 * WM * TM, BN = 16 * WN * TN, BNS = 16 * WN * TS;
    static_assert(TS == TN || (TS > TN && WN == 1), "a narrower tile than its image: one wave column only");
    using TA = TileImg<BM, AKC, NT, W>;
    using TB = TileImg<BNS, BKC, NT, W>;
    __shared__ double lds[2 * (TA::SIZE + TB::SIZE)];
    constexpr int STAGE = TA::SIZE + TB::SIZE;

    const GettProblem& p = a.p;
    const int t = threadIdx.x, lane = t & 63, wave = t >> 6;
    const int wm = wave % WM, wn = wave / WM;
    const int z = blockIdx.z, split = blockIdx.y;
    const int kbeg = split * a.kchunk;
    const int kend = min(p.K, kbeg + a.kchunk);
    const double* Ab = p.A + (p.batchA ? p.batchA[z] : 0);
    const double* Bb = p.B + (p.batchB ? p.batchB[z] : 0);

    const int ntiles_all = GRP ? a.total_tiles : a.mtiles * a.ntiles;
    const int nk = SK ? a.sk_nk : (kend - kbeg + BK - 1) / BK;
    const int nk_real = (kend - kbeg + BK - 1) / BK;
    const int sk_g0 = SK ? (int)blockIdx.x * a.sk_units : 0, sk_g1 = SK ? min(sk_g0 + a.sk_units, ntiles_all * nk) : 0;
    if (SK && sk_g0 >= sk_g1) return;
    const int sk_first = SK ? sk_g0 / nk : 0, sk_kt0 = SK ? sk_g0 - sk_first * nk : 0;
    const int ntl = SK ? (sk_g1 - 1) / nk - sk_first + 1 : (ntiles_all - (int)blockIdx.x + (int)gridDim.x - 1) / (int)gridDim.x;
    int ctile = 0;
    auto origin = [&](int j, int& m0, int& n0, int& cursor) {
        const int r0 = j * (int)gridDim.x;
        int tile = SK ? sk_first + j : r0 + xcd_remap(blockIdx.x, min((int)gridDim.x, ntiles_all - r0));
        int nt = a.ntiles;
        if (GRP) {
            while (tile >= uniform_i32(a.groups[cursor + 1].tile_start)) ++cursor;
            tile -= uniform_i32(a.groups[cursor].tile_start);
            nt = uniform_i32(a.groups[cursor].ntiles);
        }
        const int width = a.gm * nt, grp = tile / width, first = grp * a.gm;
        const int gsz = min(a.mtiles - first, a.gm), rem = tile - grp * width;
        m0 = (first + rem % gsz) * BM;
        n0 = (rem / gsz) * BN;
    };
    int fgrp = 0, cgrp = 0;

    v4d acc[TM][TN];
#pragma unroll
    for (int i = 0; i < TM; ++i)
#pragma unroll
        for (int j = 0; j < TN; ++j) acc[i][j] = (v4d){0.0, 0.0, 0.0, 0.0};

    auto store_tile = [&](int m0, int n0) {
        if (a.dbg & 1) return;
        const int nl = n0 + wn * 16 * TN + (lane & 15);
        const int ml = m0 + wm * 16 * TM + (lane >> 4);
        const int64_t* offCn = GRP ? uniform_ptr(a.groups[cgrp].offCn) : p.offCn;
        const int Ncur = GRP ? uniform_i32(a.groups[cgrp].N) : p.N;
        if (!SK && a.ksplit == 1) {
            double* Cb = p.C + (p.batchC ? p.batchC[z] : 0);
            int64_t cn[TN];
#pragma unroll
            for (int j = 0; j < TN; ++j) {
                int n = nl + 16 * j;
                cn[j] = offCn[n < Ncur ? n : Ncur - 1];
            }
#pragma unroll
            for (int i = 0; i < TM; ++i) {
                int64_t cm[4];
#pragma unroll
                for (int r = 0; r < 4; ++r) cm[r] = p.offCm[min(ml + 16 * i + 4 * r, p.M - 1)];
                double old[4][TN];
                if (p.beta != 0.0) {
#pragma unroll
                    for (int r = 0; r < 4; ++r)
#pragma unroll
                        for (int j = 0; j < TN; ++j) old[r][j] = Cb[cm[r] + cn[j]];
                }
#pragma unroll
                for (int r = 0; r < 4; ++r) {
                    if (ml + 16 * i + 4 * r >= p.M) continue;
#pragma unroll
                    for (int j = 0; j < TN; ++j) {
                        if (nl + 16 * j >= Ncur) continue;
                        double val = p.alpha * acc[i][j][r];
                        if (p.beta != 0.0) val += p.beta * old[r][j];
                        Cb[cm[r] + cn[j]] = val;
                    }
                }
            }
        } else {
            const int part = SK ? (int)blockIdx.x - (int)(((int64_t)(sk_first + ctile) * nk) / a.sk_units) : z * a.ksplit + split;
            double* slab = a.ws + (int64_t)part * (int64_t)p.M * p.N;
#pragma unroll
            for (int i = 0; i < TM; ++i)
#pragma unroll
                for (int r = 0; r < 4; ++r) {
                    int m = ml + 16 * i + 4 * r;
                    if (m >= p.M) continue;
#pragma unroll
                    for (int j = 0; j < TN; ++j) {
                        int n = nl + 16 * j;
                        if (n < p.N) slab[(int64_t)m * p.N + n] = acc[i][j][r];
                    }
                }
        }
    };

    if (nk <= 0) {
        for (int j = 0; j < ntl; ++j) {
            int m0, n0;
            origin(j, m0, n0, cgrp);
            store_tile(m0, n0);
        }
        return;
    }
    const bool ragged = RAG ? ((kend - kbeg) % BK) != 0 : false;
    const int G = SK ? sk_g1 - sk_g0 : ntl * nk;

    Stager<BM, AKC, NT, W> stA;
    Stager<BNS, BKC, NT, W> stB;
    int fkt = sk_kt0, ftile = 0, kok = sk_kt0;
    {
        int m0, n0;
        origin(0, m0, n0, fgrp);
        if (GRP) {
            const GettGroup& g = a.groups[fgrp];
            stA.init(Ab + uniform_i64(g.a_off), p.offAm, uniform_ptr(g.offAk), m0, p.M, p.K, t);
            stB.init(Bb, uniform_ptr(g.offBn), uniform_ptr(g.offBk), n0, uniform_i32(g.N), p.K, t);
        } else {
            stA.init(Ab, p.offAm, p.offAk, m0, p.M, p.K, t);
            stB.init(Bb, p.offBn, p.offBk, n0, p.N, p.K, t);
        }
    }
    auto advance_fetch = [&]() {
        if (++fkt == nk) {
            fkt = 0;
            if (++ftile < ntl) {
                int m0, n0;
                origin(ftile, m0, n0, fgrp);
                stA.rows(p.offAm, m0, p.M, t);
                if (GRP) {
                    const GettGroup& g = a.groups[fgrp];
                    stA.base = Ab + uniform_i64(g.a_off);
                    stA.offK = uniform_ptr(g.offAk);
                    stB.offK = uniform_ptr(g.offBk);
                    stB.rows(uniform_ptr(g.offBn), n0, uniform_i32(g.N), t);
                } else {
                    stB.rows(p.offBn, n0, p.N, t);
                }
            }
        }
    };
    auto next_ko = [&]() {
        stA.fetch_ko(kbeg + kok * BK, t);
        stB.fetch_ko(kbeg + kok * BK, t);
        kok = (kok + 1 == nk) ? 0 : kok + 1;
    };

    double ra0[TA::PER][W], rb0[TB::PER][W], ra1[TA::PER][W], rb1[TB::PER][W];
    next_ko();
    stA.fetch(ra0);
    stB.fetch(rb0);
    advance_fetch();
    next_ko();
    stA.stash(lds, ra0, t, kbeg + sk_kt0 * BK, kend, SK ? sk_kt0 >= nk_real - 1 : ragged && sk_kt0 == nk - 1);
    stB.stash(lds + TA::SIZE, rb0, t, kbeg + sk_kt0 * BK, kend, SK ? sk_kt0 >= nk_real - 1 : ragged && sk_kt0 == nk - 1);
    stA.fetch(ra1);
    stB.fetch(rb1);
    advance_fetch();
    next_ko();
    __syncthreads();

    const int fa = wm * 16 * TM + (lane & 15), fb = wn * 16 * TN + (lane & 15), fk = lane >> 4;
    double af0[TM], bf0[TN], af1[TM], bf1[TN];
    auto frag = [&](double (&af)[TM], double (&bf)[TN], const double* cA, const double* cB, int s) {
#pragma unroll
        for (int i = 0; i < TM; ++i) af[i] = cA[TA::at(fa + 16 * i, 4 * s + fk)];
#pragma unroll
        for (int j = 0; j < TN; ++j) bf[j] = cB[TB::at(fb + 16 * j, 4 * s + fk)];
    };
    auto mfma = [&](const double (&af)[TM], const double (&bf)[TN]) {
#pragma unroll
        for (int i = 0; i < TM; ++i)
#pragma unroll
            for (int j = 0; j < TN; ++j)
                acc[i][j] = __builtin_amdgcn_mfma_f64_16x16x4f64(af[i], bf[j], acc[i][j], 0, 0, 0);
    };
    frag(af0, bf0, lds, lds + TA::SIZE, 0);
    if (AFESP_GETT_VARIANT_ & 4) {
        if (NT == 512 && __builtin_amdgcn_readfirstlane(wave) >= 4) __builtin_amdgcn_s_setprio(1);
    } else if (NT == 512 && wave >= 4) __builtin_amdgcn_s_setprio(1);
    int kt = sk_kt0;
#ifndef AFESP_GETT_VARIANT
#define AFESP_GETT_VARIANT 0
#endif
    constexpr int VARIANT = AFESP_GETT_VARIANT;
    constexpr bool PIN = (VARIANT & 1) != 0;
    constexpr bool STAGGER = (VARIANT & 8) ? true : (VARIANT & 512) ? false : GRP;
    unsigned long long stamp_bar = 0, stamp_stash = 0, stamp_n = 0, stamp_n2 = 0;
    const unsigned long long stamp_t0 = (VARIANT & 64) ? __builtin_amdgcn_s_memtime() : 0;
#define AFESP_GETT_STASH(pa, pb)                                                                \
        if (st) {                                                                               \
            unsigned long long s0_ = 0;                                                         \
            if (VARIANT & 64) { __builtin_amdgcn_sched_barrier(0); s0_ = __builtin_amdgcn_s_memtime(); __builtin_amdgcn_sched_barrier(0); } \
            if (VARIANT & 128) { __builtin_amdgcn_s_waitcnt(0x0070); __builtin_amdgcn_sched_barrier(0); stamp_n2 += __builtin_amdgcn_s_memtime() - s0_; __builtin_amdgcn_sched_barrier(0); } \
            stA.stash(lds + (cur ^ 1) * STAGE, pa, t, kbeg + ktn * BK, kend, tail);             \
            stB.stash(lds + (cur ^ 1) * STAGE + TA::SIZE, pb, t, kbeg + ktn * BK, kend, tail);  \
            if (VARIANT & 64) { __builtin_amdgcn_sched_barrier(0); stamp_stash += __builtin_amdgcn_s_memtime() - s0_; __builtin_amdgcn_sched_barrier(0); } \
        }
#define AFESP_GETT_STEP(qa, qb, pa, pb, EARLY) AFESP_GETT_STEP_(qa, qb, pa, pb, EARLY, false)
#define AFESP_GETT_STEP_(qa, qb, pa, pb, EARLY, STEADY)                                         \
    {                                                                                           \
        const int cur = g & 1;                                                                  \
        const double* cA = lds + cur * STAGE;                                                   \
        const double* cB = cA + TA::SIZE;                                                       \
        const bool ld = (STEADY) || g + 2 < G, st = (STEADY) || g + 1 < G;                      \
        const int ktn = (kt + 1 == nk) ? 0 : kt + 1;                                            \
        const bool tail = SK ? ktn >= nk_real - 1 : ragged && (ktn == nk - 1);                  \
        if (EARLY) { AFESP_GETT_STASH(pa, pb) }                                                 \
        frag(af1, bf1, cA, cB, 1);                                                              \
        if (ld) stA.fetch(qa);                                                                  \
        mfma(af0, bf0);                                                                         \
        frag(af0, bf0, cA, cB, 2);                                                              \
        if (ld) {                                                                               \
            stB.fetch(qb);                                                                      \
            advance_fetch();                                                                    \
        }                                                                                       \
        mfma(af1, bf1);                                                                         \
        frag(af1, bf1, cA, cB, 3);                                                              \
        if (ld) next_ko();                                                                      \
        if (!(EARLY)) { AFESP_GETT_STASH(pa, pb) }                                              \
        mfma(af0, bf0);                                                                         \
        if (PIN) __builtin_amdgcn_sched_barrier(0);                                             \
        if (VARIANT & 64) {                                                                     \
            __builtin_amdgcn_sched_barrier(0);                                                  \
            const unsigned long long b0_ = __builtin_amdgcn_s_memtime();                        \
            __syncthreads();                                                                    \
            stamp_bar += __builtin_amdgcn_s_memtime() - b0_;                                    \
            ++stamp_n;                                                                          \
            __builtin_amdgcn_sched_barrier(0);                                                  \
        } else                                                                                  \
        __syncthreads();                                                                        \
        if (st) frag(af0, bf0, lds + (cur ^ 1) * STAGE, lds + (cur ^ 1) * STAGE + TA::SIZE, 0); \
        mfma(af1, bf1);                                                                         \
        if (ktn == 0) {                                                                         \
            int m0, n0;                                                                         \
            origin(ctile, m0, n0, cgrp);                                                        \
            store_tile(m0, n0);                                                                 \
            ++ctile;                                                                            \
            _Pragma("unroll") for (int i = 0; i < TM; ++i)                                      \
                _Pragma("unroll") for (int j = 0; j < TN; ++j) acc[i][j] = (v4d){0.0, 0.0, 0.0, 0.0}; \
        }                                                                                       \
        kt = ktn;                                                                               \
    }
#define AFESP_GETT_LOOP(EARLY)                                                                  \
    {                                                                                           \
        int g = 0;                                                                              \
        if (!GRP || (VARIANT & 4096))    \
            for (; g + 3 < G; g += 2) {    \
                AFESP_GETT_STEP_(ra0, rb0, ra1, rb1, EARLY, true)                               \
                ++g;                                                                            \
                AFESP_GETT_STEP_(ra1, rb1, ra0, rb0, EARLY, true)                               \
                --g;                                                                            \
            }                                                                                   \
        for (; g + 1 < G; g += 2) {                                                             \
            AFESP_GETT_STEP(ra0, rb0, ra1, rb1, EARLY)                                          \
            ++g;                                                                                \
            AFESP_GETT_STEP(ra1, rb1, ra0, rb0, EARLY)                                          \
            --g;                                                                                \
        }                                                                                       \
        if (g < G) AFESP_GETT_STEP(ra0, rb0, ra1, rb1, EARLY)                                   \
    }
    if (STAGGER && NT == 512) {
        const bool early_half = (VARIANT & 16) ? __builtin_amdgcn_readfirstlane(wave) < 4 : __builtin_amdgcn_readfirstlane(wave) >= 4;
        AFESP_GETT_LOOP(early_half)
    } else if (VARIANT & 2) {
        AFESP_GETT_LOOP(true)
    } else {
        AFESP_GETT_LOOP(false)
    }
#undef AFESP_GETT_LOOP
#undef AFESP_GETT_STASH
    if (SK && kt != 0) {
        int m0, n0;
        origin(ctile, m0, n0, cgrp);
        store_tile(m0, n0);
    }
    if ((VARIANT & 64) && lane == 0 && blockIdx.x < 256 && wave < 8 && blockIdx.y == 0 && blockIdx.z == 0) {
        unsigned long long* d = g_gett_stamp + ((int)blockIdx.x * 8 + wave) * 4;
        d[0] = __builtin_amdgcn_s_memtime() - stamp_t0;
        d[1] = stamp_bar;
        d[2] = stamp_stash;
        d[3] = (VARIANT & 128) ? (stamp_n | ((stamp_n2 / (stamp_n ? stamp_n : 1)) << 20)) : stamp_n;
    }
#undef AFESP_GETT_STEP
}

#ifndef AFESP_GETT_GROUPED_TU
__global__ __launch_bounds__(256) void gett_reduce_kernel(GettKernelArgs a)
{
    const GettProblem& p = a.p;
    const int64_t mn = (int64_t)p.M * p.N;
    const int z = blockIdx.y;
    double* Cb = p.C + (p.batchC ? p.batchC[z] : 0);
    const double* W = a.ws + (int64_t)z * a.ksplit * mn;
    const bool small = mn <= 0x7fffffff;
    for (int64_t x = (int64_t)blockIdx.x * blockDim.x + threadIdx.x; x < mn; x += (int64_t)gridDim.x * blockDim.x) {
        int m, n;
        if (small) {
            m = (int)((unsigned)x / (unsigned)p.N);
            n = (int)((unsigned)x - (unsigned)m * (unsigned)p.N);
        } else {
            m = (int)(x / p.N);
            n = (int)(x % p.N);
        }
        double* dst = Cb + p.offCm[m] + p.offCn[n];
        double s = 0.0;
        int k = 0;
        for (; k + 8 <= a.ksplit; k += 8) {
            double w[8];
#pragma unroll
            for (int q = 0; q < 8; ++q) w[q] = W[(int64_t)(k + q) * mn + x];
#pragma unroll
            for (int q = 0; q < 8; ++q) s += w[q];
        }
        for (; k < a.ksplit; ++k) s += W[(int64_t)k * mn + x];
        double val = p.alpha * s;
        if (p.beta != 0.0) val += p.beta * *dst;
        *dst = val;
    }
}

int g_dbg = 0;

template <int WM, int WN, int TM, int TN, int W>
static void preload_cfg()
{
    first_use_touch(reinterpret_cast<const void*>(gett_kernel<WM, WN, TM, TN, true, true, W>));
    first_use_touch(reinterpret_cast<const void*>(gett_kernel<WM, WN, TM, TN, true, false, W>));
    first_use_touch(reinterpret_cast<const void*>(gett_kernel<WM, WN, TM, TN, false, true, W>));
    first_use_touch(reinterpret_cast<const void*>(gett_kernel<WM, WN, TM, TN, false, false, W>));
}
void preload_gett()
{
    first_use_touch(reinterpret_cast<const void*>(gett_reduce_kernel));
    preload_cfg<2, 2, 1, 1, 1>(); preload_cfg<2, 2, 1, 2, 1>(); preload_cfg<2, 2, 1, 4, 1>();
    preload_cfg<2, 2, 2, 1, 1>(); preload_cfg<2, 2, 2, 2, 1>(); preload_cfg<2, 2, 2, 2, 2>(); preload_cfg<2, 2, 2, 4, 1>(); preload_cfg<2, 2, 2, 4, 2>();
    preload_cfg<2, 2, 4, 1, 1>(); preload_cfg<2, 2, 4, 2, 1>(); preload_cfg<2, 2, 4, 2, 2>();
    preload_cfg<2, 4, 4, 2, 1>(); preload_cfg<2, 4, 4, 2, 2>();
    preload_gett_grouped();
    preload_cfg<4, 2, 4, 4, 1>(); preload_cfg<4, 2, 4, 4, 2>(); preload_cfg<2, 4, 4, 4, 1>(); preload_cfg<2, 4, 4, 4, 2>();
    (void)hipGetLastError();
}

hipError_t gett_read_stamps(unsigned long long* out, int n)
{
    return hipMemcpyFromSymbol(out, HIP_SYMBOL(g_gett_stamp), sizeof(unsigned long long) * (size_t)(n < 256 * 8 * 4 ? n : 256 * 8 * 4));
}

#else
extern int g_dbg;
void preload_gett_grouped()
{
    first_use_touch(reinterpret_cast<const void*>(gett_kernel<2, 4, 4, 2, true, true, 2, true>));
    first_use_touch(reinterpret_cast<const void*>(gett_kernel<2, 4, 4, 2, true, true, 1, true>));
    first_use_touch(reinterpret_cast<const void*>(gett_kernel<4, 2, 4, 4, true, true, 2, true>));
    (void)hipGetLastError();
}
hipError_t gett_read_stamps_grouped(unsigned long long* out, int n)
{
    return hipMemcpyFromSymbol(out, HIP_SYMBOL(g_gett_stamp), sizeof(unsigned long long) * (size_t)(n < 256 * 8 * 4 ? n : 256 * 8 * 4));
}
#endif

template <typename Kern>
static int resident_blocks(Kern kern, int threads)
{
    int dev = 0, cus = 256, occ = 1;
    if (hipGetDevice(&dev) != hipSuccess) return cus;
    if (hipDeviceGetAttribute(&cus, hipDeviceAttributeMultiprocessorCount, dev) != hipSuccess || cus <= 0) cus = 256;
    {
        std::lock_guard<std::mutex> lk(first_use_mutex());
        if (hipOccupancyMaxActiveBlocksPerMultiprocessor(&occ, kern, threads, 0) != hipSuccess || occ <= 0) occ = 1;
    }
    return cus * occ;
}

template <int WM, int WN, int TM, int TN, bool AK, bool BK_, int W, bool GRP = false, bool RAG = !GRP, int TS = TN, bool SK = false>
static void launch_one(const GettKernelArgs& a, dim3 grid, hipStream_t st)
{
    if (SK) {
        AFESP_KLAUNCH((gett_kernel<WM, WN, TM, TN, AK, BK_, W, GRP, RAG, TS, SK>), grid, dim3(64 * WM * WN), 0, st, a);
        return;
    }
    static const int cap = resident_blocks(gett_kernel<WM, WN, TM, TN, AK, BK_, W, GRP, RAG, TS>, 64 * WM * WN);
    int per = cap / (int)(grid.y * grid.z);
    if (per < 1) per = 1;
    if (g_dbg & 2) per = 1 << 30;
    if (g_dbg & 4) per = per / 4 > 0 ? per / 4 : 1;
    if ((int)grid.x > per) grid.x = (unsigned)per;
    AFESP_KLAUNCH((gett_kernel<WM, WN, TM, TN, AK, BK_, W, GRP, RAG, TS>), grid, dim3(64 * WM * WN), 0, st, a);
}

template <int WM, int WN, int TM, int TN, int W, int TS = TN>
static void launch_cfg(const GettKernelArgs& a, dim3 grid, hipStream_t st)
{
    const bool ak = a.p.a_kcontig, bk = a.p.b_kcontig;
    if (ak && bk) launch_one<WM, WN, TM, TN, true, true, W, false, true, TS>(a, grid, st);
    else if (ak) launch_one<WM, WN, TM, TN, true, false, W, false, true, TS>(a, grid, st);
    else if (bk) launch_one<WM, WN, TM, TN, false, true, W, false, true, TS>(a, grid, st);
    else launch_one<WM, WN, TM, TN, false, false, W, false, true, TS>(a, grid, st);
}

template <int WM, int WN, int TM, int TN, int W, int TS>
static void launch_cfg_sk(const GettKernelArgs& a, dim3 grid, hipStream_t st)
{
    const bool ak = a.p.a_kcontig, bk = a.p.b_kcontig;
    if (ak && bk) launch_one<WM, WN, TM, TN, true, true, W, false, true, TS, true>(a, grid, st);
    else if (ak) launch_one<WM, WN, TM, TN, true, false, W, false, true, TS, true>(a, grid, st);
    else if (bk) launch_one<WM, WN, TM, TN, false, true, W, false, true, TS, true>(a, grid, st);
    else launch_one<WM, WN, TM, TN, false, false, W, false, true, TS, true>(a, grid, st);
}

#ifdef AFESP_GETT_GROUPED_TU
extern int g_group_m, g_allow_wide;
#else
int g_group_m = 0;
int g_force_tm = 0, g_force_tn = 0, g_force_split = 0, g_allow_wide = 1;
#define g_split_below (knobs().split_below)
#define g_split_min_steps (knobs().split_min_steps)

static int pick_t(int extent)
{
    if (extent <= 32) return 1;
    if (extent <= 64) return 2;
    return 4;
}

hipError_t gett_launch(const GettProblem& p, const GettWorkspace& ws, hipStream_t stream, int force_split, int force_tm,
                       int force_tn)
{
    if (p.M <= 0 || p.N <= 0 || p.nbatch <= 0) return hipSuccess;
    GettKernelArgs a;
    a.p = p;
    if (!force_tm) force_tm = g_force_tm;
    if (!force_tn) force_tn = g_force_tn;
    if (!force_split) force_split = g_force_split;
    const bool wide = p.wide && g_allow_wide && (p.a_kcontig || p.M % 2 == 0) && (p.b_kcontig || p.N % 2 == 0) && (p.K % 2 == 0) &&
                      p.nbatch == 1;
    int tm = force_tm ? force_tm : pick_t(p.M), tn = force_tn ? force_tn : pick_t(p.N);
    const int ksteps = (p.K + BK - 1) / BK;
    int wq_split = 0;
    if (!force_tm && !force_tn && tm == 4 && tn == 4 && wide && p.M >= 2048) {
        auto score = [&](int bm, int bn, int s, double rate, int slots) {
            const int64_t work = (int64_t)((p.M + bm - 1) / bm) * ((p.N + bn - 1) / bn) * p.nbatch * s;
            const int64_t rounds = (work + slots - 1) / slots;
            const double waste = (double)((p.M + bm - 1) / bm * bm) * ((p.N + bn - 1) / bn * bn) / ((double)p.M * p.N);
            return rate * (double)work / (double)(rounds * slots) / waste * (s > 1 ? 1.0 - 0.012 * s : 1.0);
        };
        static const int slice_opts[] = {1, 2, 3, 4, 6, 8, 12, 16};
        double best = 0.0;
        for (int big = 0; big < 2; ++big)
            for (int s : slice_opts) {
                if (s > 1 && (force_split > 0 || ksteps / s < 32)) continue;
                const double sc = score(big ? 256 : 128, 128, s, big ? 1.0 : 0.89, 256);
                if (sc > best * 1.02) { best = sc; tm = big ? 16 : 4; tn = big ? 8 : 4; wq_split = s; }
            }
        if (ksteps >= 256 || ksteps < 64)
            for (int s : slice_opts) {
                if (s > 1 && (force_split > 0 || ksteps / s < 32)) continue;
                const double sc = score(128, 64, s, ksteps >= 256 ? 0.82 : 0.97, 512);
                if (sc > best * 1.02) { best = sc; tm = 4; tn = 2; wq_split = s; }
            }
        for (int cols = 112; cols >= 96; cols -= 16)
            for (int s : slice_opts) {
                if (s > 1 && (force_split > 0 || ksteps / s < 32)) continue;
                const double sc = score(256, cols, s, 0.93, 256);
                if (sc > best * 1.02) { best = sc; tm = 16; tn = cols / 16; wq_split = s; }
            }
    }
    if (tn == 6 || tn == 7) tm = 16;
    const int BM = tm == 16 ? 256 : tm == 8 ? 128 : 32 * tm, BN = tn == 16 ? 256 : tn == 8 ? 128 : tn == 7 ? 112 : tn == 6 ? 96 : 32 * tn;
    a.mtiles = (p.M + BM - 1) / BM;
    a.ntiles = (p.N + BN - 1) / BN;
    const int64_t tiles = (int64_t)a.mtiles * a.ntiles * p.nbatch;
    int split = 1;
    if (force_split > 0) {
        split = force_split;
    } else if (wq_split > 1) {
        split = wq_split;
    } else if (tiles < g_split_below && ksteps >= 2 * g_split_min_steps) {
        split = (int)((512 + tiles - 1) / tiles);
        if (split > ksteps / g_split_min_steps) split = ksteps / g_split_min_steps;
    } else if (tiles < 1024 && ksteps >= 64 && (int64_t)p.M * p.N * 16 <= ((int64_t)p.M + p.N) * p.K) {
        split = (int)((1024 + tiles - 1) / tiles);
        if (split > ksteps / 8) split = ksteps / 8;
    }
    if (split > ksteps) split = ksteps > 0 ? ksteps : 1;
    const int64_t need = (int64_t)split * p.nbatch * p.M * p.N * (int64_t)sizeof(double);
    if (split > 1 && (ws.ptr == nullptr || (size_t)need > ws.bytes)) {
        split = (ws.ptr == nullptr) ? 1 : (int)(ws.bytes / ((size_t)p.nbatch * p.M * p.N * sizeof(double)));
        if (split < 1) split = 1;
    }
    int steps_per = (ksteps + split - 1) / split;
    if (steps_per < 1) steps_per = 1;
    a.kchunk = steps_per * BK;
    a.ksplit = (ksteps + steps_per - 1) / steps_per;
    if (a.ksplit < 1) a.ksplit = 1;
    a.ws = ws.ptr;
    a.dbg = g_dbg;
    a.groups = nullptr;
    a.total_tiles = 0;
    a.sk_units = 0;
    a.sk_nk = 0;
    a.gm = g_group_m > 0 ? g_group_m : (a.ntiles >= 8 ? 4 : a.ntiles >= 4 ? 8 : a.ntiles >= 2 ? 16 : 32);
    if (a.gm > a.mtiles) a.gm = a.mtiles;
    dim3 grid((unsigned)(a.mtiles * a.ntiles), (unsigned)a.ksplit, (unsigned)p.nbatch);
    const bool sk_off = !knobs().gett_sk;
    bool sk = false;
    if (!sk_off && tm == 16 && (tn == 6 || tn == 7) && wide && p.nbatch == 1 && force_split == 0 && a.ksplit > 1 && ksteps >= 64 && ws.ptr) {
        const int wgs = 256;
        const int64_t items = tiles * a.ksplit, rounds = (items + wgs - 1) / wgs;
        const int nkp = (ksteps + 7) / 8 * 8, j8 = (int)((tiles + 31) / 32);
        const int U = j8 * (nkp / 8);
        const int64_t total = tiles * nkp;
        const int parts = (nkp + U - 1) / U + 1;
        if ((double)items / (double)(rounds * wgs) < 0.97 && (double)tiles / (32.0 * j8) > (double)items / (double)(rounds * wgs) + 0.02 && j8 < 8 &&
            U >= 32 && parts <= 8 && (size_t)parts * p.M * p.N * sizeof(double) <= ws.bytes && total < ((int64_t)1 << 31)) {
            sk = true;
            a.sk_units = U;
            a.sk_nk = nkp;
            a.kchunk = nkp * BK;
            a.ksplit = parts;
            grid = dim3((unsigned)((total + U - 1) / U), 1, 1);
            const int always = (nkp + U - 1) / U;
            hipError_t me = hipMemsetAsync(ws.ptr + (size_t)always * p.M * p.N, 0, (size_t)(parts - always) * p.M * p.N * sizeof(double), stream);
            if (me != hipSuccess) return me;
        }
    }
    const bool gett_debug = knobs().gett_debug;
    if (gett_debug)
        fprintf(stderr, "gett_launch M %d N %d K %d batch %d akc %d bkc %d wide %d -> tm %d tn %d tiles %d x %d split %d (steps per slice %d)\n", p.M, p.N, p.K,
                p.nbatch, (int)p.a_kcontig, (int)p.b_kcontig, (int)wide, tm, tn, a.mtiles, a.ntiles, a.ksplit, a.kchunk / BK);
#define AFESP_CFG(TM_, TN_, WM_, WN_, PM_, PN_) \
    if (tm == TM_ && tn == TN_) {                                                           \
        if (wide && TM_ >= 2 && TN_ >= 2) launch_cfg<WM_, WN_, PM_, PN_, (TM_ >= 2 && TN_ >= 2) ? 2 : 1>(a, grid, stream); \
        else launch_cfg<WM_, WN_, PM_, PN_, 1>(a, grid, stream);                            \
    }
    AFESP_CFG(1, 1, 2, 2, 1, 1) AFESP_CFG(1, 2, 2, 2, 1, 2) AFESP_CFG(1, 4, 2, 2, 1, 4)
    AFESP_CFG(2, 1, 2, 2, 2, 1) AFESP_CFG(2, 2, 2, 2, 2, 2) AFESP_CFG(2, 4, 2, 2, 2, 4)
    AFESP_CFG(4, 1, 2, 2, 4, 1) AFESP_CFG(4, 2, 2, 2, 4, 2) AFESP_CFG(4, 4, 2, 4, 4, 2)
    AFESP_CFG(8, 8, 2, 2, 4, 4) AFESP_CFG(16, 8, 4, 2, 4, 4) AFESP_CFG(8, 16, 2, 4, 4, 4)
#undef AFESP_CFG
    if (sk) {
        if (tn == 7) launch_cfg_sk<8, 1, 2, 7, 2, 8>(a, grid, stream);
        else launch_cfg_sk<8, 1, 2, 6, 2, 8>(a, grid, stream);
    } else {
        if (tm == 16 && tn == 7) { if (wide) launch_cfg<8, 1, 2, 7, 2, 8>(a, grid, stream); else launch_cfg<8, 1, 2, 7, 1, 8>(a, grid, stream); }
        if (tm == 16 && tn == 6) { if (wide) launch_cfg<8, 1, 2, 6, 2, 8>(a, grid, stream); else launch_cfg<8, 1, 2, 6, 1, 8>(a, grid, stream); }
    }
    hipError_t err = hipGetLastError();
    if (err != hipSuccess) return err;
    if (a.ksplit > 1) {
        int64_t mn = (int64_t)p.M * p.N;
        unsigned gx = (unsigned)((mn + 255) / 256 > 2048 ? 2048 : (mn + 255) / 256);
        AFESP_KLAUNCH(gett_reduce_kernel, dim3(gx, (unsigned)p.nbatch), dim3(256), 0, stream, a);
        err = hipGetLastError();
    }
    return err;
}

void gett_grouped_tile(int M, bool wide, int* tm, int* tn, int* BM, int* BN)
{
    if (wide && M >= 2048) { *tm = 16; *tn = 8; *BM = 256; *BN = 128; }
    else { *tm = 4; *tn = 4; *BM = 128; *BN = 128; }
}

#endif

#ifdef AFESP_GETT_GROUPED_TU
hipError_t gett_launch_grouped(const GettProblem& p, const GettGroup* dev_groups, int ngroups, int total_tiles, int max_ntiles,
                               hipStream_t stream)
{
    if (p.M <= 0 || ngroups <= 0 || total_tiles <= 0 || p.K <= 0) return hipSuccess;
    if (p.nbatch != 1 || !p.a_kcontig || !p.b_kcontig || p.K % BK != 0) return hipErrorInvalidValue;
    GettKernelArgs a;
    a.p = p;
    const bool wide = p.wide && g_allow_wide && (p.K % 2 == 0);
    int tm, tn, BM, BN;
    gett_grouped_tile(p.M, wide, &tm, &tn, &BM, &BN);
    a.mtiles = (p.M + BM - 1) / BM;
    a.ntiles = max_ntiles;
    a.ksplit = 1;
    a.kchunk = (p.K + BK - 1) / BK * BK;
    a.ws = nullptr;
    a.dbg = g_dbg;
    a.groups = dev_groups;
    a.total_tiles = total_tiles;
    a.sk_units = 0;
    a.sk_nk = 0;
    a.gm = g_group_m > 0 ? g_group_m : std::max(1, (32 + max_ntiles / 2) / std::max(1, max_ntiles));
    if (a.gm > a.mtiles) a.gm = a.mtiles;
    dim3 grid((unsigned)total_tiles, 1, 1);
    if (tm == 16) {
        if (wide) {
            launch_one<4, 2, 4, 4, true, true, 2, true>(a, grid, stream);
        }
        else return hipErrorInvalidValue;
    } else {
        if (wide) launch_one<2, 4, 4, 2, true, true, 2, true>(a, grid, stream);
        else launch_one<2, 4, 4, 2, true, true, 1, true>(a, grid, stream);
    }
    return hipGetLastError();
}
#endif

}
```

### a-fortran-electronic-structure-program_amd/csrc/kernels.hip

```cpp
#include <algorithm>

#include "afesp_internal.h"
#include "fused.h"

namespace afesp {

namespace {
constexpr int TB = 256;
inline unsigned grid_for(int64_t n, int cap = 4096) { return (unsigned)std::max<int64_t>(1, std::min<int64_t>((n + TB - 1) / TB, cap)); }
#define GRID_STRIDE(IDX_, n) for (int64_t IDX_ = (int64_t)blockIdx.x * blockDim.x + threadIdx.x; IDX_ < (n); IDX_ += (int64_t)gridDim.x * blockDim.x)

template <int CTRL>
__device__ __forceinline__ double dpp_permuted(double v)
{
    const int lo = __builtin_amdgcn_update_dpp(0, __double2loint(v), CTRL, 0xf, 0xf, true);
    const int hi = __builtin_amdgcn_update_dpp(0, __double2hiint(v), CTRL, 0xf, 0xf, true);
    return __hiloint2double(hi, lo);
}
__device__ __forceinline__ double lane_value(double v, int from)
{
    const int lo = __builtin_amdgcn_readlane(__double2loint(v), from), hi = __builtin_amdgcn_readlane(__double2hiint(v), from);
    return __hiloint2double(hi, lo);
}
__device__ __forceinline__ double wave_sum(double v)
// ... 391 lines not shown
        fb[xa] = hcore[xa] + j - kb;
    }
}
__global__ __launch_bounds__(TB) void ump2_kernel(double* partial, unsigned* counter, double* scal, const double* __restrict__ aa,
                                                  const double* __restrict__ bb, const double* __restrict__ ab,
                                                  const double* __restrict__ ea, const double* __restrict__ eb, int n, int na, int nb)
{
    __shared__ double sm[4];
    __shared__ bool last;
    auto tri2 = [](int64_t p, int64_t q) { return p >= q ? p * (p + 1) / 2 + q : q * (q + 1) / 2 + p; };
    const int va = n - na, vb = n - nb;
    const int64_t np = (int64_t)n * (n + 1) / 2;
    const int64_t naa = (int64_t)na * na * va * va, nbb = (int64_t)nb * nb * vb * vb, nab = (int64_t)na * nb * va * vb;
    double acc[1] = {0.0};
    GRID_STRIDE(x, naa + nbb + nab)
    {
        if (x < naa + nbb) {
            const bool beta = x >= naa;
            const int o = beta ? nb : na, v = beta ? vb : va;
            const double* P = beta ? bb : aa;
            const double* e = beta ? eb : ea;
            int64_t r = beta ? x - naa : x;
            const int i = (int)(r % o);
            r /= o;
            const int j = (int)(r % o);
            r /= o;
            const int a = (int)(r % v), b = (int)(r / v);
            const double d = P[tri2(tri2(o + a, i), tri2(o + b, j))] - P[tri2(tri2(o + b, i), tri2(o + a, j))];
            acc[0] += 0.25 * d * d / (e[i] + e[j] - e[o + a] - e[o + b]);
        } else {
            int64_t r = x - naa - nbb;
            const int i = (int)(r % na);
            r /= na;
            const int a = (int)(r % va);
            r /= va;
            const int j = (int)(r % nb), b = (int)(r / nb);
            const double g = ab[tri2(na + a, i) * np + tri2(nb + b, j)];
            acc[0] += g * g / (ea[i] + eb[j] - ea[na + a] - eb[nb + b]);
        }
    }
    block_sum<1>(acc, sm);
    if (threadIdx.x == 0) {
        partial[blockIdx.x] = acc[0];
        __threadfence();
        last = atomicInc(counter, gridDim.x - 1) == gridDim.x - 1;
    }
    __syncthreads();
    if (!last) return;
    __threadfence();
    double tot[1] = {0.0};
    for (int b = threadIdx.x; b < (int)gridDim.x; b += blockDim.x) tot[0] += __builtin_nontemporal_load(&partial[b]);
    block_sum<1>(tot, sm);
    if (threadIdx.x == 0) scal[0] = tot[0];
}
}

#define LAUNCH(kernel, grid, ...)                                               \
    do {                                                                        \
        AFESP_KLAUNCH(kernel, grid, dim3(TB), 0, cx.stream, __VA_ARGS__);  \
        AFESP_HIP(hipGetLastError());                                           \
    } while (0)

void preload_kernels()
{
    first_use_touch(reinterpret_cast<const void*>(fill_kernel));
    (void)hipGetLastError();
}

void k_fill(Context& cx, double* x, int64_t n, double val)
{
    if (cx.rec) {
        if (n > 0) cx.rec->opaque({}, {frange(x, n)}, [=](Context& c_) { k_fill(c_, x, n, val); });
        return;
    }
    if (n > 0) LAUNCH(fill_kernel, dim3(grid_for(n)), x, n, val);
}
void k_copy(Context& cx, double* dst, const double* src, int64_t n)
{
    if (cx.rec) {
        const int64_t one = 1;
        if (n > 0) cx.rec->elementwise(dst, src, 1, &n, &one, &one, 1.0, 0.0);
        return;
    }
    if (n > 0) AFESP_HIP(hipMemcpyAsync(dst, src, sizeof(double) * n, hipMemcpyDeviceToDevice, cx.stream));
}
void k_axpby(Context& cx, double* y, double a, const double* x, double b, int64_t n)
{
    if (cx.rec) {
        const int64_t one = 1;
        if (n > 0) cx.rec->elementwise(y, x, 1, &n, &one, &one, a, b);
        return;
    }
    if (n > 0) LAUNCH(axpby_kernel, dim3(grid_for(n)), y, a, x, b, n);
}
void k_div(Context& cx, double* out, const double* num, const double* den, int64_t n)
{
    if (cx.rec) {
        if (n > 0) cx.rec->opaque({frange(num, n), frange(den, n)}, {frange(out, n)}, [=](Context& c_) { k_div(c_, out, num, den, n); });
        return;
    }
    if (n > 0) LAUNCH(div_kernel, dim3(grid_for(n)), out, num, den, n);
}
__global__ __launch_bounds__(256) void ivv_diag_kernel(double* ivv, const double* y, const double* x, int o, int v, int a0, int a1)
{
    const int64_t idx0 = (int64_t)blockIdx.x * blockDim.x + threadIdx.x;
    if (idx0 >= (int64_t)v * (a1 - a0)) return;
    const int64_t b = idx0 % v, a = a0 + idx0 / v, idx = b + (int64_t)v * a;
    double sy = 0.0, sx = 0.0;
    for (int m = 0; m < o; ++m) {
        sy += y[m + (int64_t)o * (b + (int64_t)v * (m + (int64_t)o * a))];
        sx += x[b + (int64_t)v * (m + (int64_t)o * (m + (int64_t)o * a))];
    }
    ivv[idx] += 2.0 * sy - sx;
}
void k_ivv_diag(Context& cx, double* ivv, const double* y, const double* x, int o, int v, int a0, int a1)
{
    if (cx.rec) throw Error(2, "k_ivv_diag: not part of a recorded sequence");
    if (a1 > a0) LAUNCH(ivv_diag_kernel, dim3(grid_for((int64_t)v * (a1 - a0))), ivv, y, x, o, v, a0, a1);
}
void k_sub(Context& cx, double* out, const double* a, const double* b, int64_t n) { if (n > 0) LAUNCH(sub_kernel, dim3(grid_for(n)), out, a, b, n); }
void k_antisym_pair(Context& cx, double* out, const double* in, int64_t d0, int64_t d1, int64_t d2, int64_t d3, int which)
{
    int64_t n = d0 * d1 * d2 * d3;
    if (n > 0) LAUNCH(antisym_pair_kernel, dim3(grid_for(n)), out, in, d0, d1, d2, d3, which);
}
void k_asym_c(Context& cx, double* asym, double* c, const double* t1, const double* t2, int o, int v)
{
    if (cx.rec) {
        const int64_t n2 = (int64_t)o * o * v * v;
        cx.rec->opaque({frange(t1, (int64_t)o * v), frange(t2, n2)}, {frange(asym, n2), frange(c, n2)},
                       [=](Context& c_) { k_asym_c(c_, asym, c, t1, t2, o, v); });
        return;
    }
    LAUNCH(asym_c_kernel, dim3(grid_for((int64_t)o * o * v * v)), asym, c, t1, t2, o, v);
}
__global__ void add_swapped_kernel(double* out, const double* y, int o, int64_t n)
{
    GRID_STRIDE(x, n)
    {
        const int i = (int)(x % o), j = (int)((x / o) % o);
        out[x] += y[x + (int64_t)(j - i) * (1 - o)];
    }
}
void k_add_swapped(Context& cx, double* out, const double* y, int o, int v)
{
    const int64_t n = (int64_t)o * o * v * v;
    LAUNCH(add_swapped_kernel, dim3(grid_for(n)), out, y, o, n);
}
void k_t2_update(Context& cx, double* t2, const double* r2, const double* r2b, const double* r2c, const double* v_oovv, const double* D2,
                 const double* pp, int o, int v, double* t1, const double* r1, const double* r1b, const double* D1, const double* r2y)
{
    if (cx.rec) {
        if (r2y) throw Error(2, "k_t2_update: the exchanged partial residual is not part of a recorded sequence");
        const int64_t n2 = (int64_t)o * o * v * v, n1 = (int64_t)o * v, np = (int64_t)o * o * ((int64_t)v * (v + 1) / 2);
        std::vector<FusedRange> rd = {frange(r2, n2), frange(v_oovv, n2), frange(D2, n2), frange(pp, np), frange(r1, n1), frange(D1, n1)};
        if (r2b) rd.push_back(frange(r2b, n2));
        if (r2c) rd.push_back(frange(r2c, n2));
        if (r1b) rd.push_back(frange(r1b, n1));
        cx.rec->opaque(rd, {frange(t2, n2), frange(t1, n1)},
                       [=](Context& c_) { k_t2_update(c_, t2, r2, r2b, r2c, v_oovv, D2, pp, o, v, t1, r1, r1b, D1); });
        return;
    }
    LAUNCH(t2_update_kernel, dim3(grid_for((int64_t)o * o * v * v)), t2, r2, r2b, r2c, v_oovv, D2, pp, o, v, t1, r1, r1b, D1, r2y);
}
__global__ void r2_full_kernel(double* out, const double* r2, const double* pp, int o, int v)
{
    const int64_t n = (int64_t)o * o * v * v;
// ... 960 lines not shown
```

### a-fortran-electronic-structure-program_amd/csrc/tgemm.hip

```cpp
#include "tgemm.h"

#include <algorithm>
#include <cstdlib>

namespace afesp {

typedef double v4d __attribute__((ext_vector_type(4)));
typedef double v2d __attribute__((ext_vector_type(2)));

constexpr int TG_STAGE = 32768;
constexpr int TG_BIMG = 16384;
constexpr int TG_SIDE = 2 * TG_STAGE;
constexpr int TG_SLOT = 4096;
constexpr int TG_NSLOT = 3;
constexpr int TG_TKT = TG_SIDE + TG_NSLOT * TG_SLOT;
constexpr int TG_LDS = TG_TKT + 64;

struct TgArgs {
    TgProblem p;
    const TgGroup* groups;
    int mtiles, gm, total_tiles;
    unsigned inv_gm, inv_gl;
    int dbg;
    unsigned* tickets;
// ... 405 lines not shown
    }
    asm volatile("s_waitcnt vmcnt(0)" ::: "memory");
#ifdef TG_STAMPS
    if (lane == 0 && blockIdx.x < 512) {
        unsigned long long* d = g_tg_stamp + ((size_t)blockIdx.x * 4 + wave) * 8;
        d[0] = __builtin_amdgcn_s_memtime() - st_t0;
        d[1] = st_bar; d[2] = st_epi; d[3] = st_steps; d[4] = st_tiles; d[5] = st_max;
        d[6] = st_t8;
        d[7] = __builtin_amdgcn_s_getreg((15 << 11) | (0 << 6) | 4);
    }
#endif
#undef TG_MF
#undef TG_SB
#undef TG_FRAG
#undef TG_DMA
}

__global__ __launch_bounds__(256, 2) void tgemm_kernel(TgArgs a) { tgemm_body<false>(a); }
__global__ __launch_bounds__(256, 2) void tgemm_ring_kernel(TgArgs a) { tgemm_body<false>(a); }
__global__ __launch_bounds__(256, 2) void tgemm_xform_kernel(TgArgs a) { tgemm_body<false>(a); }
__global__ __launch_bounds__(256, 2) void tgemm_mixed_kernel(TgArgs a) { tgemm_body<true>(a); }

unsigned tgemm_inverse(int d) { return d <= 1 ? 0u : (unsigned)(((uint64_t)1 << 32) / (unsigned)d + 1); }
int tgemm_group_m(int M, int max_ntiles, int bm)
{
    const int mtiles = (M + bm - 1) / bm;
    if (mtiles <= 4) return mtiles;
    const int patch = knobs().tg_patch;
    return std::min(mtiles, std::max(1, (patch + max_ntiles / 2) / std::max(1, max_ntiles)));
}

void preload_tgemm()
{
    first_use_touch(reinterpret_cast<const void*>(tgemm_kernel));
    first_use_touch(reinterpret_cast<const void*>(tgemm_mixed_kernel));
    first_use_touch(reinterpret_cast<const void*>(tgemm_ring_kernel));
    first_use_touch(reinterpret_cast<const void*>(tgemm_xform_kernel));
    (void)hipGetLastError();
}

void tgemm_state_free(TgLaunchState& st)
{
    if (st.tickets) (void)hipFree(st.tickets);
    st.tickets = nullptr;
}

hipError_t tgemm_launch(const TgProblem& p, const TgGroup* dev_groups, int ngroups, int total_tiles, int max_ntiles, hipStream_t stream,
                        TgLaunchState& st, int bm)
{
    if (p.M <= 0 || ngroups <= 0 || total_tiles <= 0) return hipSuccess;
    if (bm != 0 && bm != 96 && bm != TG_BM) return hipErrorInvalidValue;
    const bool mixed = bm != 0;
    int& cap = mixed ? st.cap_mixed : st.cap;
    if (cap == 0) {
        int dev = 0, cus = 256, occ = 2;
        if (hipGetDevice(&dev) == hipSuccess) {
            if (hipDeviceGetAttribute(&cus, hipDeviceAttributeMultiprocessorCount, dev) != hipSuccess || cus <= 0) cus = 256;
            std::lock_guard<std::mutex> lk(first_use_mutex());
            if (hipOccupancyMaxActiveBlocksPerMultiprocessor(&occ, mixed ? tgemm_mixed_kernel : tgemm_kernel, 256, 0) != hipSuccess || occ <= 0) occ = 2;
        }
        cap = cus * occ;
    }
    TgArgs a;
    a.p = p;
    a.groups = dev_groups;
    a.bm = mixed ? bm : TG_BM;
    a.mtiles = (p.M + a.bm - 1) / a.bm;
    a.total_tiles = total_tiles;
    a.dbg = knobs().tg_dbg;
    a.gm = tgemm_group_m(p.M, max_ntiles, a.bm);
    a.inv_gm = tgemm_inverse(a.gm);
    a.inv_gl = tgemm_inverse(std::max(1, a.mtiles % a.gm));
    const int grid_env = knobs().tg_grid;
    const unsigned grid = (unsigned)std::min(total_tiles, grid_env > 0 ? grid_env : cap);
    const int prio_env = knobs().tg_prio_shift;
    a.prio_shift = (int64_t)total_tiles >= (int64_t)2 * grid ? prio_env : 0;
    const bool dyn_env = knobs().tg_dynamic != 0;
    const bool dyn_force = knobs().tg_dynamic == 2;
    a.tickets = nullptr;
    a.chunk = (int)(grid / 8);
    a.inv_chunk = tgemm_inverse(a.chunk);
    if (dyn_env && grid % 8 == 0 && ((int64_t)total_tiles >= (int64_t)4 * grid || dyn_force)) {
        if (!st.tickets && hipMalloc((void**)&st.tickets, 64) != hipSuccess) return hipErrorOutOfMemory;
        const hipError_t me = hipMemsetAsync(st.tickets, 0, 64, stream);
        if (me != hipSuccess) return me;
        a.tickets = st.tickets;
    }
    if (mixed) AFESP_KLAUNCH(tgemm_mixed_kernel, dim3(grid), dim3(256), 0, stream, a);
    else if (p.tag == 1) AFESP_KLAUNCH(tgemm_ring_kernel, dim3(grid), dim3(256), 0, stream, a);
    else if (p.tag == 2) AFESP_KLAUNCH(tgemm_xform_kernel, dim3(grid), dim3(256), 0, stream, a);
    else AFESP_KLAUNCH(tgemm_kernel, dim3(grid), dim3(256), 0, stream, a);
    ++(mixed ? st.launches_mixed : st.launches);
    return hipGetLastError();
}

}
```

### include/afesp.h

```cpp
#ifndef AFESP_H
#define AFESP_H
#include <stdint.h>

#ifdef __cplusplus
extern "C" {
#endif

typedef struct afesp_ctx afesp_ctx;

int afesp_ctx_create(int device, afesp_ctx** out);
void afesp_ctx_destroy(afesp_ctx* ctx);
const char* afesp_last_error(const afesp_ctx* ctx);
int afesp_version(void);
int64_t afesp_neri(int64_t nbasis);

int afesp_ao2mo_mp2(afesp_ctx* ctx, int64_t nbasis, int64_t nocc, const double* canon_coeff, const double* canon_levels,
                    const double* eri_packed, double* eri_mo_packed, double* e_mp2);

int afesp_mo_window(afesp_ctx* ctx, int64_t nbasis, int64_t nocc, int64_t n_frozen_core, int64_t n_frozen_virt,
                    const double* canon_levels, const double* eri_mo_packed, double* eri_act, double* e_mp2);

int afesp_ccsd_init(afesp_ctx* ctx, int64_t nocc, int64_t nvirt, const double* eri_mo_packed, const double* canon_levels,
                    int diis_n_errmat);

int afesp_ccsd_iterate(afesp_ctx* ctx, double e_tol, double t_tol, double* energy, double* rms_sq, int* converged);
int afesp_ccsd_energy(afesp_ctx* ctx, double e_tol, double t_tol, double* energy, double* rms_sq, int* converged);
int afesp_ccsd_diis(afesp_ctx* ctx);
int afesp_ccsd_solve(afesp_ctx* ctx, int maxiter, double e_tol, double t_tol, double* iter_energy, double* iter_rms_sq,
                     int* niter);
int afesp_ccsd_get_amplitudes(afesp_ctx* ctx, double* t1, double* t2);
int afesp_ccsd_set_amplitudes(afesp_ctx* ctx, const double* t1, const double* t2);
int afesp_ccsd_get_tensor(afesp_ctx* ctx, const char* name, double* out, int64_t capacity);
int afesp_ccsd_update_intermediates(afesp_ctx* ctx);
int afesp_ccsd_update_amplitudes(afesp_ctx* ctx);

int64_t afesp_ccsd_t_ntriples(int64_t nocc);
int afesp_ccsd_t(afesp_ctx* ctx, int64_t t_begin, int64_t t_end, double out[4]);
int afesp_ccsd_t_shard_bounds(afesp_ctx* ctx, int64_t nocc, int64_t nvirt, int cr, int world, int64_t* bounds);
int afesp_ccsd_t_plain(afesp_ctx* ctx, int64_t t_begin, int64_t t_end, double out[2]);

int afesp_ccsd_cr_intermediates(afesp_ctx* ctx);
int afesp_ccsd_t_cr(afesp_ctx* ctx, int64_t t_begin, int64_t t_end, double out[6]);

int afesp_read_eri_text(afesp_ctx* ctx, const char* path, int64_t nbasis, double* eri_packed, int64_t* nread);
int afesp_set_eri(afesp_ctx* ctx, int64_t nbasis, const double* eri_packed);
int afesp_build_fock(afesp_ctx* ctx, int64_t nbasis, const double* density, const double* core_hamil, double* fock);
int afesp_write_fcidump(afesp_ctx* ctx, const char* path, int64_t nbasis, int64_t* nwritten);

#define AFESP_SO_FOO_AS_PUBLISHED 1
int afesp_ccsd_so_init(afesp_ctx* ctx, int64_t nbasis, int64_t nel, const double* eri_mo_packed, const double* canon_levels,
                       int diis_n_errmat, int flags);
int afesp_ccsd_so_energy(afesp_ctx* ctx, double e_tol, double t_tol, double* energy, double* rms_sq, int* converged);
int afesp_ccsd_so_iterate(afesp_ctx* ctx, double e_tol, double t_tol, double* energy, double* rms_sq, int* converged);
int afesp_ccsd_so_diis(afesp_ctx* ctx);
int afesp_ccsd_so_get_amplitudes(afesp_ctx* ctx, double* t1, double* t2);
int afesp_ccsd_so_set_amplitudes(afesp_ctx* ctx, const double* t1, const double* t2);
int afesp_ccsd_so_get_tensor(afesp_ctx* ctx, const char* name, double* out, int64_t capacity);
int64_t afesp_ccsd_so_t_ntriples(int64_t nocc);
int afesp_ccsd_so_t(afesp_ctx* ctx, int64_t t_begin, int64_t t_end, double* e_t);

int afesp_build_fock_uhf(afesp_ctx* ctx, int64_t nbasis, const double* dens_a, const double* dens_b, const double* core_hamil,
                         double* fock_a, double* fock_b);
int afesp_ao2mo_ump2(afesp_ctx* ctx, int64_t nbasis, int64_t nalpha, int64_t nbeta, const double* coeff_a, const double* coeff_b,
                     const double* levels_a, const double* levels_b, const double* eri_packed, double* eri_aa, double* eri_ab,
                     double* eri_bb, double* e_ump2);
int afesp_ccsd_uso_init(afesp_ctx* ctx, int64_t nbasis, int64_t nalpha, int64_t nbeta, const double* levels_a, const double* levels_b,
                        int diis_n_errmat);
int afesp_umo_window(afesp_ctx* ctx, int64_t nbasis, int64_t nalpha, int64_t nbeta, int64_t n_frozen_core, int64_t n_frozen_virt,
                     const double* levels_a, const double* levels_b, double* eri_aa, double* eri_ab, double* eri_bb, double* e_ump2);

int afesp_mp2_vv_density(afesp_ctx* ctx, int64_t nbasis, int64_t nocc, int64_t n_frozen_core, const double* canon_levels, double* d_vv,
                         double* e_mp2);
int afesp_ump2_vv_density(afesp_ctx* ctx, int64_t nbasis, int64_t nalpha, int64_t nbeta, int64_t n_frozen_core, const double* levels_a,
                          const double* levels_b, double* d_a, double* d_b, double* e_ump2);

#define AFESP_COMM_RCCL 0
#define AFESP_COMM_HOST 1
int afesp_device_count(void);
int afesp_comm_unique_id(char id_out[128]);
int afesp_comm_init(afesp_ctx* ctx, int rank, int world, int transport, const char* bootstrap_path, const char* unique_id);
int afesp_comm_destroy(afesp_ctx* ctx);
int afesp_allreduce_sum(afesp_ctx* ctx, double* inout, int64_t n);
int afesp_ccsd_set_split(afesp_ctx* ctx, int mode);
int afesp_ccsd_is_split(afesp_ctx* ctx, int* split);
int afesp_ccsd_set_fused(afesp_ctx* ctx, int mode);
int afesp_ccsd_iteration_launches(afesp_ctx* ctx, int* launches);
int afesp_ccsd_t_block_size(afesp_ctx* ctx, int64_t nocc, int64_t nvirt, int cr, int* block_size);

int afesp_arena_stats(afesp_ctx* ctx, double out[4]);

int afesp_test_inject(afesp_ctx* ctx, int what);
int afesp_launch_counts(afesp_ctx* ctx, uint64_t out[4]);
uint64_t afesp_first_use_count(void);
int afesp_test_ring_path(int64_t nocc, int64_t nvirt);
int afesp_debug_stamps(unsigned long long* out, int n);

int afesp_gemm(afesp_ctx* ctx, char transA, char transB, int64_t m, int64_t n, int64_t k, double alpha, const double* A,
               const double* B, double beta, double* C);
int afesp_permute4(afesp_ctx* ctx, const int64_t dims[4], const char order[4], const double* in, double* out, int has_beta,
                   double beta);
int afesp_contract(afesp_ctx* ctx, double alpha, const double* A, const char* la, const int64_t* dimsA, const double* B,
                   const char* lb, const int64_t* dimsB, double beta, double* C, const char* lc, const int64_t* dimsC,
                   int force_split, int force_tm, int force_tn);

int afesp_synthetic_init(afesp_ctx* ctx, int64_t nocc, int64_t nvirt, double scale, uint64_t seed, int diis_n_errmat);
int afesp_synthetic_ao(afesp_ctx* ctx, int64_t nbasis, double scale, uint64_t seed);
int afesp_ccsd_pp_ladder_flop(afesp_ctx* ctx, double* flop);
int afesp_ccsd_iteration_flop(afesp_ctx* ctx, double* flop);
int afesp_time_pp_ladder(afesp_ctx* ctx, int reps, double* ms_per_launch);
int afesp_bench_stream(afesp_ctx* ctx, int64_t n, int reps, double* ms_per_launch);
int afesp_bench_contract(afesp_ctx* ctx, const char* la, const int64_t* dimsA, const char* lb, const int64_t* dimsB,
                         const char* lc, const int64_t* dimsC, int reps, double* ms_per_launch);
int afesp_profile(afesp_ctx* ctx, int enable, double out[8]);
int afesp_set_tuning(int group_m, int force_tm, int force_tn, int force_split);

#ifdef __cplusplus
}
#endif
#endif
```

Baseline: 59.74 TFLOP/s.

## Fuse split-K reduction into GETT kernel via last-arriver tile counters

Removes the separate gett_reduce_kernel launch and the stream-K slab memset. Each split-K workgroup now bumps a per-tile atomic counter after writing its slab, and the last arriver sums the slabs into C inside the same kernel. Counters live in a reserved 64 KiB prefix of the workspace and are zeroed when lanes are set up. The grid is clamped so that each block owns at most 64 tiles, which fits the tile bitmask. A launch-counting API is added alongside. The cost is extra atomics and fences plus a serialized tail combine in the last block for each tile.

```diff
diff --git a/a-fortran-electronic-structure-program_amd/afesp_amd/capi.py b/a-fortran-electronic-structure-program_amd/afesp_amd/capi.py
--- a/a-fortran-electronic-structure-program_amd/afesp_amd/capi.py
+++ b/a-fortran-electronic-structure-program_amd/afesp_amd/capi.py
@@ -26,7 +26,7 @@
     "afesp_device_count", "afesp_comm_unique_id", "afesp_comm_init", "afesp_comm_destroy", "afesp_allreduce_sum",
     "afesp_build_fock_uhf", "afesp_ao2mo_ump2", "afesp_ccsd_uso_init", "afesp_mo_window", "afesp_umo_window",
     "afesp_mp2_vv_density", "afesp_ump2_vv_density",
-    "afesp_ccsd_t_block_size", "afesp_test_inject", "afesp_ccsd_is_split", "afesp_ccsd_set_split", "afesp_ccsd_set_fused", "afesp_ccsd_iteration_launches", "afesp_debug_stamps", "afesp_launch_counts", "afesp_first_use_count", "afesp_test_ring_path", "afesp_arena_stats",
+    "afesp_ccsd_t_block_size", "afesp_test_inject", "afesp_ccsd_is_split", "afesp_ccsd_set_split", "afesp_ccsd_set_fused", "afesp_ccsd_iteration_launches", "afesp_debug_stamps", "afesp_launch_counts", "afesp_launch_count", "afesp_first_use_count", "afesp_test_ring_path", "afesp_arena_stats",
 ]
 COMM_RCCL, COMM_HOST = 0, 1
 
@@ -120,6 +120,7 @@
     L.afesp_ccsd_iteration_launches.argtypes = [C.c_void_p, C.POINTER(C.c_int)]
     L.afesp_debug_stamps.argtypes = [C.c_void_p, C.c_int]
     L.afesp_launch_counts.argtypes = [C.c_void_p, C.POINTER(C.c_uint64)]
+    L.afesp_launch_count.argtypes = [C.c_void_p, C.POINTER(C.c_uint64)]
     L.afesp_first_use_count.argtypes = []
     L.afesp_first_use_count.restype = C.c_uint64
     L.afesp_test_ring_path.argtypes = [C.c_int64, C.c_int64]
@@ -290,6 +291,11 @@
         out = (C.c_uint64 * 4)()
         self._chk(self.L.afesp_launch_counts(self.h, out))
         return dict(tall=int(out[0]), gett=int(out[1]), tgemm=int(out[2]), tgemm_mixed=int(out[3]))
+
+    def launch_count(self):
+        n = C.c_uint64()
+        self._chk(self.L.afesp_launch_count(self.h, C.byref(n)))
+        return int(n.value)
 
     def ccsd_set_split(self, mode):
         self._chk(self.L.afesp_ccsd_set_split(self.h, int(mode)))
diff --git a/a-fortran-electronic-structure-program_amd/csrc/afesp_internal.h b/a-fortran-electronic-structure-program_amd/csrc/afesp_internal.h
--- a/a-fortran-electronic-structure-program_amd/csrc/afesp_internal.h
+++ b/a-fortran-electronic-structure-program_amd/csrc/afesp_internal.h
@@ -83,6 +83,7 @@
     GettWorkspace ws{nullptr, 0};
     TgLaunchState tg;
     unsigned long long n_tall = 0, n_gett = 0;
+    unsigned long long n_launches = 0;
     bool in_repack = false;
     GettProblem* capture = nullptr;
     struct Lane {
diff --git a/a-fortran-electronic-structure-program_amd/csrc/capi.hip b/a-fortran-electronic-structure-program_amd/csrc/capi.hip
--- a/a-fortran-electronic-structure-program_amd/csrc/capi.hip
+++ b/a-fortran-electronic-structure-program_amd/csrc/capi.hip
@@ -66,6 +66,7 @@
     if (!c) return 1;
     Context& cx = c->cx;
     first_use_tls_device() = cx.device;
+    launch_counter_tls() = &cx.n_launches;
     knobs_refresh();
     auto failed = [&](const char* what, int code) {
         cx.last_error = what;
@@ -286,6 +287,7 @@
 {
     if (!ctx) return;
     first_use_tls_device() = ctx->cx.device;
+    launch_counter_tls() = nullptr;
     (void)hipSetDevice(ctx->cx.device);
     if (ctx->cx.startup.joinable()) ctx->cx.startup.join();
     ctx->cc_programs_reset();
@@ -1128,6 +1130,14 @@
     });
 }
 
+int afesp_launch_count(afesp_ctx* ctx, uint64_t* count)
+{
+    return entry(ctx, [&](Context& cx) {
+        if (!count) throw Error(1, "afesp_launch_count: null argument");
+        *count = cx.n_launches;
+    });
+}
+
 int afesp_arena_stats(afesp_ctx* ctx, double out[4])
 {
     return entry(ctx, [&](Context& cx) {
diff --git a/a-fortran-electronic-structure-program_amd/csrc/ccsd.hip b/a-fortran-electronic-structure-program_amd/csrc/ccsd.hip
--- a/a-fortran-electronic-structure-program_amd/csrc/ccsd.hip
+++ b/a-fortran-electronic-structure-program_amd/csrc/ccsd.hip
@@ -320,6 +320,7 @@
         Tensor osh = view(cx.scratch("ooov_sh", s.I_ooov_p.size()), {(int64_t)s.o, (int64_t)s.o, (int64_t)s.o, (int64_t)s.v});
         if (v1 > v0) {
             if (s.pp_sym) {
+                count_launch();
                 AFESP_HIP(hipMemsetAsync(osh.d + osh.stride[3] * v0, 0, sizeof(double) * osh.stride[3] * (v1 - v0), cx.stream));
                 ccsd_ooov_pair_form(cx, s, osh.d, v0, v1);
             } else {
@@ -507,6 +508,7 @@
     if (sh) {
         r2s.d = s.r2_sh;
         const int64_t np = (int64_t)s.v * (s.v + 1) / 2;
+        count_launch();
         AFESP_HIP(hipMemsetAsync(s.pp, 0, sizeof(double) * ((int64_t)s.o * s.o * np + s.r2.size() + s.r1.size()), cx.stream));
     }
     if (par) {
@@ -778,6 +780,7 @@
 void diis_check_flag(Context& cx, const double* host_scal)
 {
     if (host_scal[DIIS_FLAG_SLOT] != 0.0) {
+        count_launch();
         AFESP_HIP(hipMemsetAsync(cx.scal + DIIS_FLAG_SLOT, 0, sizeof(double), cx.stream));
         throw Error(4, "ccsd::update_diis_cc: Linear solve failed!");
     }
diff --git a/a-fortran-electronic-structure-program_amd/csrc/contract.hip b/a-fortran-electronic-structure-program_amd/csrc/contract.hip
--- a/a-fortran-electronic-structure-program_amd/csrc/contract.hip
+++ b/a-fortran-electronic-structure-program_amd/csrc/contract.hip
@@ -216,12 +216,16 @@
         lanes[0].ws = ws;
         AFESP_HIP(hipEventCreateWithFlags(&fork_ev, hipEventDisableTiming));
     }
+    auto zero_counters = [&](const GettWorkspace& w) { AFESP_HIP(hipMemsetAsync(w.ptr, 0, GETT_WS_COUNTER_BYTES, lanes[0].stream)); };
     if (lanes.size() == 1 && !prepared.lanes.empty()) {
         if (prepared.ws_block) {
             arena.live[prepared.ws_block] = prepared.ws_bytes;
             owned.push_back(prepared.ws_block);
         }
-        for (Lane& l : prepared.lanes) lanes.push_back(l);
+        for (Lane& l : prepared.lanes) {
+            zero_counters(l.ws);
+            lanes.push_back(l);
+        }
         prepared.lanes.clear();
         prepared.ws_block = nullptr;
     }
@@ -231,6 +235,7 @@
             owned.push_back(p);
             lanes[i].ws.ptr = (double*)p;
             lanes[i].ws.bytes = lane_ws_bytes;
+            zero_counters(lanes[i].ws);
         }
     while ((int)lanes.size() < nlanes) {
         Lane l;
@@ -240,6 +245,7 @@
         void* p = arena.get(l.ws.bytes);
         owned.push_back(p);
         l.ws.ptr = (double*)p;
+        zero_counters(l.ws);
         lanes.push_back(l);
     }
     AFESP_HIP(hipEventRecord(fork_ev, lanes[0].stream));
@@ -353,6 +359,7 @@
     hipStreamCaptureStatus st = hipStreamCaptureStatusNone;
     if (n > 64 || !cx.res_dev || hipStreamIsCapturing(cx.stream, &st) != hipSuccess || st != hipStreamCaptureStatusNone) {
         (void)hipGetLastError();
+        count_launch();
         AFESP_HIP(hipMemcpyAsync(cx.scal_host, cx.scal, sizeof(double) * n, hipMemcpyDeviceToHost, cx.stream));
         cx.sync();
         return cx.scal_host;
diff --git a/a-fortran-electronic-structure-program_amd/csrc/first_use.h b/a-fortran-electronic-structure-program_amd/csrc/first_use.h
--- a/a-fortran-electronic-structure-program_amd/csrc/first_use.h
+++ b/a-fortran-electronic-structure-program_amd/csrc/first_use.h
@@ -37,6 +37,15 @@
     first_use_touch(fn);
     seen.fetch_or(bit, std::memory_order_release);
 }
+inline unsigned long long*& launch_counter_tls()
+{
+    static thread_local unsigned long long* p = nullptr;
+    return p;
+}
+inline void count_launch()
+{
+    if (unsigned long long* p = launch_counter_tls()) ++*p;
+}
 inline std::atomic<uint64_t>& first_use_count()
 {
     static std::atomic<uint64_t> n{0};
@@ -53,5 +62,6 @@
             ::afesp::first_use_resolve(reinterpret_cast<const void*>(kernel), afesp_seen_, afesp_bit_);                 \
             ::afesp::first_use_count().fetch_add(1, std::memory_order_relaxed);                                         \
         }                                                                                                               \
+        ::afesp::count_launch();                                                                                        \
         kernel<<<(grid), (block), (shmem), (stream)>>>(__VA_ARGS__);                                                    \
     } while (0)
diff --git a/a-fortran-electronic-structure-program_amd/csrc/fused.hip b/a-fortran-electronic-structure-program_amd/csrc/fused.hip
--- a/a-fortran-electronic-structure-program_amd/csrc/fused.hip
+++ b/a-fortran-electronic-structure-program_amd/csrc/fused.hip
@@ -231,7 +231,7 @@
         std::vector<FusedRange> rd = {frange(g.A, a_span), frange(g.B, b_span)};
         if (g.beta != 0.0) rd.push_back(frange(g.C, c_span));
         const GettProblem gp = g;
-        opaque(rd, {frange(g.C, c_span)}, [gp](Context& c) { AFESP_HIP(gett_launch(gp, c.ws, c.stream)); }, 2);
+        opaque(rd, {frange(g.C, c_span)}, [gp](Context& c) { AFESP_HIP(gett_launch(gp, c.ws, c.stream)); });
         ops.back().heavy = true;
         return;
     }
diff --git a/a-fortran-electronic-structure-program_amd/csrc/gett.h b/a-fortran-electronic-structure-program_amd/csrc/gett.h
--- a/a-fortran-electronic-structure-program_amd/csrc/gett.h
+++ b/a-fortran-electronic-structure-program_amd/csrc/gett.h
@@ -38,6 +38,7 @@
 hipError_t gett_launch_grouped(const GettProblem& p, const GettGroup* dev_groups, int ngroups, int total_tiles, int max_ntiles,
                                hipStream_t stream);
 
+constexpr size_t GETT_WS_COUNTER_BYTES = (size_t)64 << 10;
 struct GettWorkspace {
     double* ptr;
     size_t bytes;
diff --git a/a-fortran-electronic-structure-program_amd/csrc/gett.hip b/a-fortran-electronic-structure-program_amd/csrc/gett.hip
--- a/a-fortran-electronic-structure-program_amd/csrc/gett.hip
+++ b/a-fortran-electronic-structure-program_amd/csrc/gett.hip
@@ -116,6 +116,7 @@
     int ksplit;
     int kchunk;
     double* ws;
+    unsigned* cnt;
     int mtiles, ntiles;
     int gm;
     int dbg;
@@ -124,6 +125,46 @@
     int sk_units;
     int sk_nk;
 };
+
+template <int UE, int UK, int BM, int BN, int NT>
+__device__ __forceinline__ void combine_slabs(const GettProblem& p, double* Cb, const double* slabs, int64_t mn, int pieces, int m0, int n0, int t)
+{
+    for (int e0 = t; e0 < BM * BN; e0 += NT * UE) {
+        int64_t off[UE], coff[UE];
+        bool ok[UE];
+        double s[UE];
+#pragma unroll
+        for (int u = 0; u < UE; ++u) {
+            const int e = e0 + u * NT, m = m0 + e / BN, n = n0 + e % BN;
+            ok[u] = e < BM * BN && m < p.M && n < p.N;
+            off[u] = ok[u] ? (int64_t)m * p.N + n : 0;
+            coff[u] = ok[u] ? p.offCm[m] + p.offCn[n] : 0;
+            s[u] = 0.0;
+        }
+        for (int k0 = 0; k0 < pieces; k0 += UK) {
+            double x[UE][UK];
+#pragma unroll
+            for (int q = 0; q < UK; ++q)
+#pragma unroll
+                for (int u = 0; u < UE; ++u) x[u][q] = (k0 + q < pieces) ? slabs[(int64_t)(k0 + q) * mn + off[u]] : 0.0;
+#pragma unroll
+            for (int q = 0; q < UK; ++q)
+#pragma unroll
+                for (int u = 0; u < UE; ++u) s[u] += x[u][q];
+        }
+        double old[UE];
+        if (p.beta != 0.0) {
+#pragma unroll
+            for (int u = 0; u < UE; ++u) old[u] = Cb[coff[u]];
+        }
+#pragma unroll
+        for (int u = 0; u < UE; ++u) {
+            double val = p.alpha * s[u];
+            if (p.beta != 0.0) val += p.beta * old[u];
+            if (ok[u]) Cb[coff[u]] = val;
+        }
+    }
+}
 
 __device__ __forceinline__ int xcd_remap(int b, int nwg)
 {
@@ -174,6 +215,8 @@
         n0 = (rem / gsz) * BN;
     };
     int fgrp = 0, cgrp = 0;
+    unsigned long long last_mask = 0;
+    int flag_buf = 0;
 
     v4d acc[TM][TN];
 #pragma unroll
@@ -220,8 +263,12 @@
                 }
             }
         } else {
-            const int part = SK ? (int)blockIdx.x - (int)(((int64_t)(sk_first + ctile) * nk) / a.sk_units) : z * a.ksplit + split;
-            double* slab = a.ws + (int64_t)part * (int64_t)p.M * p.N;
+            const int sk_w0 = SK ? (int)(((int64_t)(sk_first + ctile) * nk) / a.sk_units) : 0;
+            const int pieces = SK ? (int)(((int64_t)(sk_first + ctile + 1) * nk - 1) / a.sk_units) - sk_w0 + 1 : a.ksplit;
+            const int part = SK ? (int)blockIdx.x - sk_w0 : split;
+            const int64_t mn = (int64_t)p.M * p.N;
+            double* slabs = a.ws + (SK ? (int64_t)0 : (int64_t)z * a.ksplit * mn);
+            double* slab = slabs + (int64_t)part * mn;
 #pragma unroll
             for (int i = 0; i < TM; ++i)
 #pragma unroll
@@ -234,6 +281,42 @@
                         if (n < p.N) slab[(int64_t)m * p.N + n] = acc[i][j][r];
                     }
                 }
+            const int r0t = ctile * (int)gridDim.x;
+            const int tile = SK ? sk_first + ctile : r0t + xcd_remap(blockIdx.x, min((int)gridDim.x, ntiles_all - r0t));
+            unsigned* cnt = a.cnt + ((int64_t)z * ntiles_all + tile);
+            volatile unsigned* word = reinterpret_cast<volatile unsigned*>(lds + flag_buf * STAGE);
+            asm volatile("s_waitcnt vmcnt(0)" ::: "memory");
+            __syncthreads();
+            if (t == 0) {
+                __builtin_amdgcn_fence(__ATOMIC_RELEASE, "agent");
+                asm volatile("s_waitcnt vmcnt(0)" ::: "memory");
+                const bool last = __hip_atomic_fetch_add(cnt, 1u, __ATOMIC_RELAXED, __HIP_MEMORY_SCOPE_AGENT) == (unsigned)(pieces - 1);
+                if (last) __hip_atomic_store(cnt, 0u, __ATOMIC_RELAXED, __HIP_MEMORY_SCOPE_AGENT);
+                *word = last ? 1u : 0u;
+            }
+            __syncthreads();
+            if (__builtin_amdgcn_readfirstlane((int)*word) != 0) last_mask |= 1ull << ctile;
+            __syncthreads();
+        }
+    };
+    auto combine_tiles = [&]() {
+        if (last_mask == 0) return;
+        if (t == 0) {
+            __builtin_amdgcn_fence(__ATOMIC_ACQUIRE, "agent");
+            asm volatile("s_waitcnt vmcnt(0)" ::: "memory");
+        }
+        __syncthreads();
+        double* Cb = p.C + (p.batchC ? p.batchC[z] : 0);
+        const int64_t mn = (int64_t)p.M * p.N;
+        const double* slabs = a.ws + (SK ? (int64_t)0 : (int64_t)z * a.ksplit * mn);
+        for (int j = 0; j < 64 && (last_mask >> j) != 0; ++j) {
+            if (!((last_mask >> j) & 1)) continue;
+            int m0, n0, grp = 0;
+            origin(j, m0, n0, grp);
+            const int sk_w0 = SK ? (int)(((int64_t)(sk_first + j) * nk) / a.sk_units) : 0;
+            const int pieces = SK ? (int)(((int64_t)(sk_first + j + 1) * nk - 1) / a.sk_units) - sk_w0 + 1 : a.ksplit;
+            if (pieces <= 4) combine_slabs<8, 4, BM, BN, NT>(p, Cb, slabs, mn, pieces, m0, n0, t);
+            else combine_slabs<4, 8, BM, BN, NT>(p, Cb, slabs, mn, pieces, m0, n0, t);
         }
     };
 
@@ -377,6 +460,7 @@
         if (ktn == 0) {                                                                         \
             int m0, n0;                                                                         \
             origin(ctile, m0, n0, cgrp);                                                        \
+            flag_buf = cur;                                                                     \
             store_tile(m0, n0);                                                                 \
             ++ctile;                                                                            \
             _Pragma("unroll") for (int i = 0; i < TM; ++i)                                      \
@@ -417,6 +501,7 @@
         origin(ctile, m0, n0, cgrp);
         store_tile(m0, n0);
     }
+    if (!GRP) combine_tiles();
     if ((VARIANT & 64) && lane == 0 && blockIdx.x < 256 && wave < 8 && blockIdx.y == 0 && blockIdx.z == 0) {
         unsigned long long* d = g_gett_stamp + ((int)blockIdx.x * 8 + wave) * 4;
         d[0] = __builtin_amdgcn_s_memtime() - stamp_t0;
@@ -428,40 +513,6 @@
 }
 
 #ifndef AFESP_GETT_GROUPED_TU
-__global__ __launch_bounds__(256) void gett_reduce_kernel(GettKernelArgs a)
-{
-    const GettProblem& p = a.p;
-    const int64_t mn = (int64_t)p.M * p.N;
-    const int z = blockIdx.y;
-    double* Cb = p.C + (p.batchC ? p.batchC[z] : 0);
-    const double* W = a.ws + (int64_t)z * a.ksplit * mn;
-    const bool small = mn <= 0x7fffffff;
-    for (int64_t x = (int64_t)blockIdx.x * blockDim.x + threadIdx.x; x < mn; x += (int64_t)gridDim.x * blockDim.x) {
-        int m, n;
-        if (small) {
-            m = (int)((unsigned)x / (unsigned)p.N);
-            n = (int)((unsigned)x - (unsigned)m * (unsigned)p.N);
-        } else {
-            m = (int)(x / p.N);
-            n = (int)(x % p.N);
-        }
-        double* dst = Cb + p.offCm[m] + p.offCn[n];
-        double s = 0.0;
-        int k = 0;
-        for (; k + 8 <= a.ksplit; k += 8) {
-            double w[8];
-#pragma unroll
-            for (int q = 0; q < 8; ++q) w[q] = W[(int64_t)(k + q) * mn + x];
-#pragma unroll
-            for (int q = 0; q < 8; ++q) s += w[q];
-        }
-        for (; k < a.ksplit; ++k) s += W[(int64_t)k * mn + x];
-        double val = p.alpha * s;
-        if (p.beta != 0.0) val += p.beta * *dst;
-        *dst = val;
-    }
-}
-
 int g_dbg = 0;
 
 template <int WM, int WN, int TM, int TN, int W>
@@ -474,7 +525,6 @@
 }
 void preload_gett()
 {
-    first_use_touch(reinterpret_cast<const void*>(gett_reduce_kernel));
     preload_cfg<2, 2, 1, 1, 1>(); preload_cfg<2, 2, 1, 2, 1>(); preload_cfg<2, 2, 1, 4, 1>();
     preload_cfg<2, 2, 2, 1, 1>(); preload_cfg<2, 2, 2, 2, 1>(); preload_cfg<2, 2, 2, 2, 2>(); preload_cfg<2, 2, 2, 4, 1>(); preload_cfg<2, 2, 2, 4, 2>();
     preload_cfg<2, 2, 4, 1, 1>(); preload_cfg<2, 2, 4, 2, 1>(); preload_cfg<2, 2, 4, 2, 2>();
@@ -529,6 +579,7 @@
     if (per < 1) per = 1;
     if (g_dbg & 2) per = 1 << 30;
     if (g_dbg & 4) per = per / 4 > 0 ? per / 4 : 1;
+    if (a.ksplit > 1 && per < ((int)grid.x + 63) / 64) per = ((int)grid.x + 63) / 64;
     if ((int)grid.x > per) grid.x = (unsigned)per;
     AFESP_KLAUNCH((gett_kernel<WM, WN, TM, TN, AK, BK_, W, GRP, RAG, TS>), grid, dim3(64 * WM * WN), 0, st, a);
 }
@@ -628,9 +679,12 @@
         if (split > ksteps / 8) split = ksteps / 8;
     }
     if (split > ksteps) split = ksteps > 0 ? ksteps : 1;
+    const bool ws_ok = ws.ptr != nullptr && ws.bytes > GETT_WS_COUNTER_BYTES && tiles <= (int64_t)(GETT_WS_COUNTER_BYTES / sizeof(unsigned));
+    const size_t slab_bytes = ws_ok ? ws.bytes - GETT_WS_COUNTER_BYTES : 0;
+    double* const slab_ptr = ws_ok ? ws.ptr + GETT_WS_COUNTER_BYTES / sizeof(double) : nullptr;
     const int64_t need = (int64_t)split * p.nbatch * p.M * p.N * (int64_t)sizeof(double);
-    if (split > 1 && (ws.ptr == nullptr || (size_t)need > ws.bytes)) {
-        split = (ws.ptr == nullptr) ? 1 : (int)(ws.bytes / ((size_t)p.nbatch * p.M * p.N * sizeof(double)));
+    if (split > 1 && (!ws_ok || (size_t)need > slab_bytes)) {
+        split = !ws_ok ? 1 : (int)(slab_bytes / ((size_t)p.nbatch * p.M * p.N * sizeof(double)));
         if (split < 1) split = 1;
     }
     int steps_per = (ksteps + split - 1) / split;
@@ -638,7 +692,8 @@
     a.kchunk = steps_per * BK;
     a.ksplit = (ksteps + steps_per - 1) / steps_per;
     if (a.ksplit < 1) a.ksplit = 1;
-    a.ws = ws.ptr;
+    a.ws = slab_ptr;
+    a.cnt = reinterpret_cast<unsigned*>(ws.ptr);
     a.dbg = g_dbg;
     a.groups = nullptr;
     a.total_tiles = 0;
@@ -649,7 +704,7 @@
     dim3 grid((unsigned)(a.mtiles * a.ntiles), (unsigned)a.ksplit, (unsigned)p.nbatch);
     const bool sk_off = !knobs().gett_sk;
     bool sk = false;
-    if (!sk_off && tm == 16 && (tn == 6 || tn == 7) && wide && p.nbatch == 1 && force_split == 0 && a.ksplit > 1 && ksteps >= 64 && ws.ptr) {
+    if (!sk_off && tm == 16 && (tn == 6 || tn == 7) && wide && p.nbatch == 1 && force_split == 0 && a.ksplit > 1 && ksteps >= 64 && ws_ok) {
         const int wgs = 256;
         const int64_t items = tiles * a.ksplit, rounds = (items + wgs - 1) / wgs;
         const int nkp = (ksteps + 7) / 8 * 8, j8 = (int)((tiles + 31) / 32);
@@ -657,16 +712,13 @@
         const int64_t total = tiles * nkp;
         const int parts = (nkp + U - 1) / U + 1;
         if ((double)items / (double)(rounds * wgs) < 0.97 && (double)tiles / (32.0 * j8) > (double)items / (double)(rounds * wgs) + 0.02 && j8 < 8 &&
-            U >= 32 && parts <= 8 && (size_t)parts * p.M * p.N * sizeof(double) <= ws.bytes && total < ((int64_t)1 << 31)) {
+            U >= 32 && parts <= 8 && (size_t)parts * p.M * p.N * sizeof(double) <= slab_bytes && total < ((int64_t)1 << 31)) {
             sk = true;
             a.sk_units = U;
             a.sk_nk = nkp;
             a.kchunk = nkp * BK;
             a.ksplit = parts;
             grid = dim3((unsigned)((total + U - 1) / U), 1, 1);
-            const int always = (nkp + U - 1) / U;
-            hipError_t me = hipMemsetAsync(ws.ptr + (size_t)always * p.M * p.N, 0, (size_t)(parts - always) * p.M * p.N * sizeof(double), stream);
-            if (me != hipSuccess) return me;
         }
     }
     const bool gett_debug = knobs().gett_debug;
@@ -690,15 +742,7 @@
         if (tm == 16 && tn == 7) { if (wide) launch_cfg<8, 1, 2, 7, 2, 8>(a, grid, stream); else launch_cfg<8, 1, 2, 7, 1, 8>(a, grid, stream); }
         if (tm == 16 && tn == 6) { if (wide) launch_cfg<8, 1, 2, 6, 2, 8>(a, grid, stream); else launch_cfg<8, 1, 2, 6, 1, 8>(a, grid, stream); }
     }
-    hipError_t err = hipGetLastError();
-    if (err != hipSuccess) return err;
-    if (a.ksplit > 1) {
-        int64_t mn = (int64_t)p.M * p.N;
-        unsigned gx = (unsigned)((mn + 255) / 256 > 2048 ? 2048 : (mn + 255) / 256);
-        AFESP_KLAUNCH(gett_reduce_kernel, dim3(gx, (unsigned)p.nbatch), dim3(256), 0, stream, a);
-        err = hipGetLastError();
-    }
-    return err;
+    return hipGetLastError();
 }
 
 void gett_grouped_tile(int M, bool wide, int* tm, int* tn, int* BM, int* BN)
@@ -725,6 +769,7 @@
     a.ksplit = 1;
     a.kchunk = (p.K + BK - 1) / BK * BK;
     a.ws = nullptr;
+    a.cnt = nullptr;
     a.dbg = g_dbg;
     a.groups = dev_groups;
     a.total_tiles = total_tiles;
diff --git a/a-fortran-electronic-structure-program_amd/csrc/kernels.hip b/a-fortran-electronic-structure-program_amd/csrc/kernels.hip
--- a/a-fortran-electronic-structure-program_amd/csrc/kernels.hip
+++ b/a-fortran-electronic-structure-program_amd/csrc/kernels.hip
@@ -497,7 +497,10 @@
         if (n > 0) cx.rec->elementwise(dst, src, 1, &n, &one, &one, 1.0, 0.0);
         return;
     }
-    if (n > 0) AFESP_HIP(hipMemcpyAsync(dst, src, sizeof(double) * n, hipMemcpyDeviceToDevice, cx.stream));
+    if (n > 0) {
+        count_launch();
+        AFESP_HIP(hipMemcpyAsync(dst, src, sizeof(double) * n, hipMemcpyDeviceToDevice, cx.stream));
+    }
 }
 void k_axpby(Context& cx, double* y, double a, const double* x, double b, int64_t n)
 {
diff --git a/a-fortran-electronic-structure-program_amd/csrc/tgemm.hip b/a-fortran-electronic-structure-program_amd/csrc/tgemm.hip
--- a/a-fortran-electronic-structure-program_amd/csrc/tgemm.hip
+++ b/a-fortran-electronic-structure-program_amd/csrc/tgemm.hip
@@ -511,6 +511,7 @@
     a.inv_chunk = tgemm_inverse(a.chunk);
     if (dyn_env && grid % 8 == 0 && ((int64_t)total_tiles >= (int64_t)4 * grid || dyn_force)) {
         if (!st.tickets && hipMalloc((void**)&st.tickets, 64) != hipSuccess) return hipErrorOutOfMemory;
+        count_launch();
         const hipError_t me = hipMemsetAsync(st.tickets, 0, 64, stream);
         if (me != hipSuccess) return me;
         a.tickets = st.tickets;
diff --git a/include/afesp.h b/include/afesp.h
--- a/include/afesp.h
+++ b/include/afesp.h
@@ -91,6 +91,7 @@
 
 int afesp_test_inject(afesp_ctx* ctx, int what);
 int afesp_launch_counts(afesp_ctx* ctx, uint64_t out[4]);
+int afesp_launch_count(afesp_ctx* ctx, uint64_t* count);
 uint64_t afesp_first_use_count(void);
 int afesp_test_ring_path(int64_t nocc, int64_t nvirt);
 int afesp_debug_stamps(unsigned long long* out, int n);
```

Result: no change. 59.58 TFLOP/s (-0.3%).
